# marcemq/crowdmod-ddpm-4D

Hardware: AMD Instinct MI355X
Metric: denoise-steps/sec (UNet fwd + sampler update) at ATC [B,4,T,H,W] (higher is better)
Workload: dtype f32; 1 GPU; config/ATC.yml sampling on the 12x36 grid, fp32 arithmetic (fp32 matrix instructions; fp32 products built from f16 two-way splits -- three v_mfma_f32_32x32x16_f16 cross terms, fp32 accumulate, same error against the reference as round 3's six-term bf16 form -- in the Winograd / quarter-resolution / last-conv layers, whose input is GroupNorm + SiLU output, and in the upsample layers, whose raw inpu; channels=4, past_len=5, future_len=3, global_batch=64, parallelism=batch-shard x1 (2 stream lanes of 32 chains per rank)

## Files before the change

### crowdmod-ddpm-4d_amd/csrc/cm_attn_block.hip

```cpp
#include "cm_kernels.h"

#include <algorithm>

namespace cm {

typedef float f32x4 __attribute__((ext_vector_type(4)));

constexpr int ATT_NT = 768;
constexpr int ATT_KS = 3;

template <int D>
__global__ __launch_bounds__(ATT_NT) void attn_head_kernel(const AttnBlockArgs a) {
  constexpr int NT = ATT_NT, NW = NT / 64;
  constexpr int KD = D < 16 ? 16 : D;
  constexpr int DS = KD + 4;
  constexpr int NBQ = (D + 15) / 16;
  constexpr int NBT = 3 * NBQ;
  constexpr int PARTS = D / 8;
  constexpr int E = 4 * D;
  constexpr int XS = E + 8;
  constexpr int Q4 = E >> 2;
  constexpr int RL = NT / Q4;
  extern __shared__ __attribute__((aligned(16))) float sm[];
  const int S = a.S;
  float *Xs = sm;
  float *Wi = Xs + (size_t)S * XS;
  float *Wo = Wi + (size_t)NBT * 16 * XS;
  float *Qs = Wo + (size_t)E * DS;
  float *Ks = Qs + (size_t)S * DS;
  float *Vs = Ks + (size_t)S * DS;
  float *bi = Vs + (size_t)S * DS;
  float *red = bi + NBT * 16;
  const int h = blockIdx.x, b = blockIdx.y, tid = threadIdx.x;
  const int lane = tid & 63, wave = __builtin_amdgcn_readfirstlane(tid >> 6);
  const int r16 = lane & 15, kq = lane >> 4;

  const int q4 = tid % Q4, rl = tid / Q4;
  const float *xb = a.x + (size_t)b * S * E;
  constexpr int UX = 3;
  constexpr int NWI = (NBT * 16 + RL - 1) / RL;
  constexpr int NWO = (E * (KD / 4) + NT - 1) / NT;
  f32x4 vx[UX], vwi[NWI], vwo[NWO];
#pragma unroll
  for (int u = 0; u < UX; ++u) vx[u] = *reinterpret_cast<const f32x4 *>(xb + (size_t)min(rl + u * RL, S - 1) * E + 4 * q4);
#pragma unroll
  for (int u = 0; u < NWI; ++u) {
    const int wr = min(rl + u * RL, NBT * 16 - 1);
    const int which = wr / (NBQ * 16), c = min(wr % (NBQ * 16), D - 1);
    vwi[u] = *reinterpret_cast<const f32x4 *>(a.w_in + (size_t)(which * E + h * D + c) * E + 4 * q4);
  }
#pragma unroll
  for (int u = 0; u < NWO; ++u) {
    const int i = min(tid + u * NT, E * (KD / 4) - 1);
    const int n = i / (KD / 4), c4 = min(i % (KD / 4), D / 4 - 1);
    vwo[u] = *reinterpret_cast<const f32x4 *>(a.w_out + (size_t)n * E + h * D + 4 * c4);
  }
  const f32x4 ga = *reinterpret_cast<const f32x4 *>(a.gamma + 4 * q4);
  const f32x4 be = *reinterpret_cast<const f32x4 *>(a.beta + 4 * q4);
  float bval = 0.f;
  {
    const int tb = min(tid, NBT * 16 - 1);
    const int which = tb / (NBQ * 16), c = min(tb % (NBQ * 16), D - 1);
    bval = a.b_in[which * E + h * D + c];
  }
  float s1 = 0.f;
#pragma unroll
  for (int u = 0; u < UX; ++u) {
    const int row = rl + u * RL;
    if (row < S) {
      *reinterpret_cast<f32x4 *>(Xs + row * XS + 4 * q4) = vx[u];
      s1 += (vx[u][0] + vx[u][1]) + (vx[u][2] + vx[u][3]);
    }
  }
#pragma unroll
  for (int u = 0; u < NWI; ++u) {
    const int wr = rl + u * RL;
    if (wr < NBT * 16) *reinterpret_cast<f32x4 *>(Wi + wr * XS + 4 * q4) = vwi[u];
  }
#pragma unroll
  for (int u = 0; u < NWO; ++u) {
    const int i = tid + u * NT;
    if (i < E * (KD / 4)) {
      const int n = i / (KD / 4), c4 = i % (KD / 4);
      *reinterpret_cast<f32x4 *>(Wo + n * DS + 4 * c4) = (4 * c4 < D) ? vwo[u] : f32x4{0.f, 0.f, 0.f, 0.f};
    }
// ... 133 lines not shown
        float L = 0.f;
        f32x4 O0 = {0.f, 0.f, 0.f, 0.f}, O1 = {0.f, 0.f, 0.f, 0.f};
#pragma unroll
        for (int s2i = 0; s2i < ATT_KS; ++s2i) {
          const float *mp = mrg + ((prow * ATT_KS + s2i) * PARTS + part) * 12;
          const float w = (mp[1] > 0.f) ? __expf(mp[0] - M) : 0.f;
          L += mp[1] * w;
          O0 += *reinterpret_cast<const f32x4 *>(mp + 4) * w;
          O1 += *reinterpret_cast<const f32x4 *>(mp + 8) * w;
        }
        const float inv = 1.0f / L;
        *reinterpret_cast<f32x4 *>(Qs + row * DS + 8 * part) = O0 * inv;
        *reinterpret_cast<f32x4 *>(Qs + row * DS + 8 * part + 4) = O1 * inv;
      }
      __syncthreads();
    }
  }

  {
    constexpr int NJ = KD / 16;
    constexpr int nbe = E >> 4;
    float *pout = a.part + ((size_t)h * a.B + b) * (size_t)S * E;
    for (int item = wave; item < nmb * nbe; item += NW) {
      const int mb = item / nbe, nb = item - mb * nbe;
      const int arow = min(mb * 16 + r16, S - 1);
      f32x4 af[NJ], bf[NJ];
#pragma unroll
      for (int j = 0; j < NJ; ++j) {
        af[j] = *reinterpret_cast<const f32x4 *>(Qs + arow * DS + 16 * j + 4 * kq);
        bf[j] = *reinterpret_cast<const f32x4 *>(Wo + (nb * 16 + r16) * DS + 16 * j + 4 * kq);
      }
      f32x4 acc = {0.f, 0.f, 0.f, 0.f};
#pragma unroll
      for (int j = 0; j < NJ; ++j)
#pragma unroll
        for (int jj = 0; jj < 4; ++jj) acc = __builtin_amdgcn_mfma_f32_16x16x4f32(af[j][jj], bf[j][jj], acc, 0, 0, 0);
      const int n = nb * 16 + r16;
#pragma unroll
      for (int reg = 0; reg < 4; ++reg) {
        const int row = mb * 16 + 4 * kq + reg;
        if (row < S) pout[(size_t)row * E + n] = acc[reg];
      }
    }
  }
}

size_t attn_block_lds_bytes(int S, int E, int heads) {
  const int D = E / heads, KD = D < 16 ? 16 : D, NBT = 3 * ((D + 15) / 16);
  return ((size_t)S * (E + 8) + (size_t)NBT * 16 * (E + 8) + (size_t)E * (KD + 4) + (size_t)3 * S * (KD + 4) + (size_t)NBT * 16 +
          (size_t)(ATT_NT / (E / 4)) * 8 + 8) * sizeof(float);
}

bool attn_block_ok(int S, int E, int heads, int groups) {
  if (heads != 4 || E % heads) return false;
  const int D = E / heads;
  if (D != 8 && D != 16 && D != 32) return false;
  if (groups != 8 || E % (4 * groups)) return false;
  return S >= 1 && attn_block_lds_bytes(S, E, heads) <= 160 * 1024;
}

hipError_t launch_attn_block(const AttnBlockArgs &a, hipStream_t st) {
  if (!attn_block_ok(a.S, a.E, a.heads, a.groups)) return hipErrorInvalidValue;
  const int D = a.E / a.heads;
  const size_t smem = attn_block_lds_bytes(a.S, a.E, a.heads);
#define CM_ATTNB(DD)                                                                                        \
  if (D == DD) {                                                                                            \
    static bool attr_set[64] = {false};                                                                     \
    int dev = 0;                                                                                            \
    (void)hipGetDevice(&dev);                                                                               \
    if (!attr_set[dev & 63]) {                                                                              \
      hipError_t e = hipFuncSetAttribute(reinterpret_cast<const void *>(attn_head_kernel<DD>),              \
                                         hipFuncAttributeMaxDynamicSharedMemorySize, 160 * 1024);           \
      if (e != hipSuccess) return e;                                                                        \
      attr_set[dev & 63] = true;                                                                            \
    }                                                                                                       \
    hipLaunchKernelGGL((attn_head_kernel<DD>), dim3(a.heads, a.B), dim3(ATT_NT), smem, st, a);                 \
    return hipGetLastError();                                                                               \
  }
  CM_ATTNB(8) CM_ATTNB(16) CM_ATTNB(32)
#undef CM_ATTNB
  return hipErrorInvalidValue;
}

}
```

### crowdmod-ddpm-4d_amd/csrc/cm_kernels.h

```cpp
#pragma once
#include <hip/hip_runtime.h>
#include <stdint.h>
#include <stdlib.h>
#include <vector>

namespace cm {

inline const char *diag_env(const char *name) {
  static const bool on = [] { const char *d = getenv("CM_DIAG"); return d && d[0] == '1' && d[1] == 0; }();
  return on ? getenv(name) : nullptr;
}

#ifdef __HIPCC__
typedef float cm_f32x2_t __attribute__((ext_vector_type(2)));
typedef float cm_f32x4_t __attribute__((ext_vector_type(4)));
typedef __bf16 cm_bf16x2_t __attribute__((ext_vector_type(2)));
typedef unsigned cm_u32x2_t __attribute__((ext_vector_type(2)));
typedef _Float16 cm_f16x4_t __attribute__((ext_vector_type(4)));
__device__ __forceinline__ unsigned cm_cvt_pk_bf16(float a, float b) {
  const cm_f32x2_t v = {a, b};
  return __builtin_bit_cast(unsigned, __builtin_convertvector(v, cm_bf16x2_t));
}
template <int NT = 3>
__device__ __forceinline__ void cm_split3_bf16(cm_f32x4_t x, cm_u32x2_t (&t)[3]) {
// ... 213 lines not shown
  float h2_oscale;
  const float *wq;
  const float *bias;
  const float *temb;
  int temb_stride;
  const long long *tidx;
  const float *resid;
  int res_cs;
  float *out;
  int out_cs, Co, B, Y, X;
  float *stat_part, *stat_cnt;
  int stat_C;
  const float *s2src0, *s2src1;
  int s2C0, s2C1;
  const float *s2w;
  int qshift;
  const float *pm;
  int pm_stride;
  int raw;
};
bool conv_qr_ok(const QrArgs &a);
bool conv_qr2_b6_ok(const QrArgs &a);
hipError_t launch_qr_b6_repack(const float *wq, float *wq6, long long n_floats, int Ci, hipStream_t st);
hipError_t launch_conv_qr(const QrArgs &a, hipStream_t st);

bool conv_f16d_pick(int Z, int Y, int X, int *bz, int *by, int *bx, int *mbw);
bool conv_f16d_ok(const ConvArgs &a, int mbw);
int conv_f16d_slots(const ConvArgs &a, int mbw);
hipError_t launch_conv_f16d(const ConvArgs &a, int mbw, hipStream_t st);

bool conv_fin_pick(int Y, int X, int *by, int *bx);
bool conv_fin_ok(const ConvArgs &a);
struct StepArgs;
bool conv_fin_fuse_ok(const ConvArgs &a, const StepArgs &s);
hipError_t launch_conv_fin(const ConvArgs &a, const float *wfin, int mode , hipStream_t st,
                           const StepArgs *step = nullptr, int variant = 1);
inline int conv_first_const_ztiles(int bz, int ntz, int P) {
  if (bz < 1 || P < 2 || (P - 1) % bz) return 0;
  const int n = (P - 1) / bz;
  return n < ntz ? n : 0;
}
hipError_t launch_fin_pack(const float *w_ref , float *wfin, int Co, int mode , hipStream_t st, float wscale = 1.f);
constexpr size_t CM_FIN_W_FLOATS = 4 * 2 * 3 * 64 * 4;

hipError_t launch_chan_stats(const float *x, int B, int V, int C, int nslice, float *part, float *cnt, hipStream_t st);
hipError_t launch_gn_finalize(const float *part0, const float *cnt0, int ns0, int C0, const float *part1,
                              const float *cnt1, int ns1, int C1, int V, const float *gamma, const float *beta,
                              int groups, float eps, float *gn, float *mr, int B, hipStream_t st);
struct CombineArgs {
  const float *part; int S; long long stride;
  const float *bias; const float *temb; int temb_stride; const long long *tidx;
  const float *resid; int res_cs;
  float *out; int C, V, B;
  float *stat_part; float *stat_cnt; int nslots;
  const float *fin_gamma, *fin_beta; float *fin_gn, *fin_mr;
  const float *fin_p1, *fin_n1; int fin_ns1, fin_C1, fin_groups; float fin_eps;
};
hipError_t launch_ksplit_combine(const CombineArgs &a, hipStream_t st);
bool combine_gn_ok(const CombineArgs &a);
hipError_t launch_combine_gn(const CombineArgs &a, hipStream_t st);
hipError_t launch_assemble_input(const float *past, const float *future, float *x8, int B, int C, int H, int W,
                                 int P, int F, int which , hipStream_t st);
hipError_t launch_extract_output(const float *eps_cl, int cs, float *out, int B, int C, int H, int W, int P, int F,
                                 hipStream_t st);
hipError_t launch_time_mlp(const float *table, const float *W1, const float *b1, const float *W2, const float *b2,
                           const float *Wd, const float *bd, int te, int tx, int nproj, int nrows, float *temb_raw,
                           float *out, const long long *rowidx, hipStream_t st);
hipError_t launch_attn_core(const float *qkv, float *out, int B, int S, int E, int heads, hipStream_t st);
hipError_t launch_attn_core_f16(const float *qkv, float *out, int B, int S, int E, int heads, hipStream_t st);

struct AttnBlockArgs {
  const float *x;
  const float *gamma, *beta;
  const float *w_in, *b_in;
  const float *w_out;
  float *part;
  int B, S, E, heads, groups;
  float eps;
};
bool attn_block_ok(int S, int E, int heads, int groups);
size_t attn_block_lds_bytes(int S, int E, int heads);
hipError_t launch_attn_block(const AttnBlockArgs &a, hipStream_t st);

enum { DIT_PRO_NONE = 0, DIT_PRO_LN = 1, DIT_PRO_PATCH = 2 };
enum { DIT_EPI_BIAS = 0, DIT_EPI_SILU = 1, DIT_EPI_SILU2 = 2, DIT_EPI_GELU = 3, DIT_EPI_GATE = 4, DIT_EPI_PATCH = 5,
       DIT_EPI_UNPATCH = 6 };
struct DitGemmArgs {
  int pro, epi;
  const float *A; int lda;
  const float *W, *bias;
  float *Y; int ldy;
  long long M; int N, K;
  int grp, grp_stride, grp_off;
  int a_compact;
  int tok;
  const long long *tbuf;
  const float *mod; int ldmod;
  int off_shift, off_scale, off_gate;
  const float *x8;
  const float *spos, *tpos;
  int L, Hh, Ww, p, pt, Ns, wpn, Cout;
};
struct DitAttnArgs {
  const float *qkv;
  float *out;
  int B, Tp, Ns, qs, E, heads;
};
hipError_t launch_dit_gemm(const DitGemmArgs &a, hipStream_t st);
hipError_t launch_dit_attn_spatial(const DitAttnArgs &a, hipStream_t st);
hipError_t launch_dit_attn_temporal(const DitAttnArgs &a, hipStream_t st);
hipError_t launch_dit_attn_full(const DitAttnArgs &a, hipStream_t st);

struct StepRow { int t; float c_x, c_eps, c_noise, guid; int draw; int step; float mass; };
struct StepArgs {
  float *x;
  const float *eps_cl;
  int cs;
  float *x8;
  const float *noise;
  float *hist;
  int B, C, H, W, P, F;
  float c_x, c_eps, c_noise;
  float guid;
  unsigned long long seed;
  long long sample_id_base;
  int step;
  int draw;
  const StepRow *tab; const int *kctr;
  long long row_stride;
  long long boff;
  long long *t_next; long long t_next_v;
};
hipError_t launch_sampler_step(const StepArgs &a, hipStream_t st);
#ifdef __HIPCC__
__device__ __forceinline__ void philox4x32_10(unsigned c0, unsigned c1, unsigned c2, unsigned c3, unsigned k0,
                                              unsigned k1, unsigned out[4]) {
#pragma unroll
  for (int i = 0; i < 10; ++i) {
    const unsigned long long p0 = 0xD2511F53ull * c0;
    const unsigned long long p1 = 0xCD9E8D57ull * c2;
    const unsigned n0 = (unsigned)(p1 >> 32) ^ c1 ^ k0;
    const unsigned n1 = (unsigned)p1;
    const unsigned n2 = (unsigned)(p0 >> 32) ^ c3 ^ k1;
    const unsigned n3 = (unsigned)p0;
    c0 = n0; c1 = n1; c2 = n2; c3 = n3;
    k0 += 0x9E3779B9u;
    k1 += 0xBB67AE85u;
  }
  out[0] = c0; out[1] = c1; out[2] = c2; out[3] = c3;
}

__device__ __forceinline__ float philox_normal(unsigned long long seed, long long sample, int step, long long elem) {
  unsigned r[4];
  philox4x32_10((unsigned)(elem >> 1), (unsigned)sample, (unsigned)step, (unsigned)((sample >> 32) ^ 0x5eed),
                (unsigned)seed, (unsigned)(seed >> 32), r);
  const float u1 = ((float)(r[0] >> 8) + 0.5f) * (1.0f / 16777216.0f);
  const float u2 = ((float)(r[1] >> 8) + 0.5f) * (1.0f / 16777216.0f);
  const float rad = sqrtf(-2.0f * __logf(u1));
  const float ang = 6.283185307179586f * u2;
  return (elem & 1) ? rad * __sinf(ang) : rad * __cosf(ang);
}

__device__ __forceinline__ void cm_step_resolve(StepArgs &a) {
  if (a.tab) {
    const int k = *a.kctr;
    const StepRow r = a.tab[k];
// ... 132 lines not shown
```

### crowdmod-ddpm-4d_amd/csrc/cm_model.cpp

```cpp
#include <hip/hip_runtime.h>

#include <algorithm>
#include <cmath>
#include <cstdarg>
#include <cstdio>
#include <cstring>
#include <map>
#include <memory>
#include <set>
#include <string>
#include <thread>
#include <vector>

#include "../../include/crowdmod_hip.h"
#include "cm_kernels.h"

namespace {

thread_local std::string g_err;

int fail(const char *fmt, ...) {
  char buf[1024];
  va_list ap;
  va_start(ap, fmt);
// ... 47 lines not shown
  std::string prefix;
  int cin, cout, attention, skip, level;
};

enum OpKind { OP_CONV, OP_STATS, OP_GNFIN, OP_ATTN, OP_ATTNBLK };

struct Op {
  OpKind kind;
  int cls;
  cm::ConvArgs ca{};
  int MB = 1, NB = 1;
  int *d_hvtab = nullptr, *d_mtab = nullptr;
  Act *stat_act = nullptr;
  int pm_off = -1;
  const Act *in0 = nullptr, *in1 = nullptr;
  std::string wname, bname;
  int temb_off = -1;
  int gn_op = -1;
  int ref_taps = 1;
  int ks = 1;
  const Act *skip0 = nullptr, *skip1 = nullptr;
  std::string skip_w, skip_b;
  float *d_s2w = nullptr, *d_bias_fused = nullptr;
  bool skip_if_fused = false;
  bool wino = false;
  float *d_wwino = nullptr;
  float *d_wwino16 = nullptr;
  float *d_wwino_b6 = nullptr;
  long long wwino_floats = 0;
  float *d_wfrag16 = nullptr;
  float *d_w1x1_16 = nullptr;
  long long wpar_stride16 = 0;
  bool f16d = false;
  int f16d_bz = 0, f16d_by = 0, f16d_bx = 0, f16d_mbw = 0;
  bool ups = false;
  int ups_tz = 0, ups_ty = 0, ups_tx = 0, ups_mbw = 0, ups_planes = 0;
  float *d_wups16 = nullptr;
  long long wups16_stride = 0;
  float *d_wups_b6 = nullptr;
  long long wups_b6_stride = 0;
  float *d_w16d = nullptr, *d_w16d_skip = nullptr;
  bool h2_off = false;
  bool dbg_h2 = false;
  bool dbg_raw = false;
  float *d_wfin_h2 = nullptr, *d_wwino_h2 = nullptr, *d_wqr_h2 = nullptr;
  float *d_wups_h2 = nullptr;
  float h2_oscale = 1.f;
  bool qr = false;
  float *d_wqr = nullptr, *d_wqr_skip = nullptr;
  float *d_wqr_b6 = nullptr;
  bool train_qr = false;
  long long wqr_floats = 0;
  bool qr_consumer = false;
  bool first_k = false;
  int first_cin = 4;
  float *d_wfirst = nullptr;
  bool small_n = false;
  float *d_wsmall = nullptr;
  int small_nco = 4;
  bool fin = false;
  int fin_by = 0, fin_bx = 0;
  float *d_wfin = nullptr, *d_wfin16 = nullptr, *d_wfin_src = nullptr;
  float *d_zero_bias = nullptr;
  const Act *out_act = nullptr, *resid_act = nullptr;
  double flops_per_sample = 0;
  std::string label;
  double prof_ms = 0;
  int64_t prof_n = 0;
  const Act *act = nullptr;
  const Act *g0 = nullptr, *g1 = nullptr;
  const float *gamma = nullptr, *beta = nullptr;
  float *gn_out = nullptr;
  float *gn_mr = nullptr;
  std::string gname, bename;
  const float *qkv = nullptr;
  float *aout = nullptr;
  int S = 0, E = 0;
  bool in_attn_block = false;
  const Act *ab_x = nullptr;
  Act *ab_out = nullptr;
  int ab_gn = -1, ab_qkv = -1, ab_outc = -1;
  float *d_win = nullptr, *d_wout = nullptr;
  std::string win_name, wout_name;
};

enum ConvKernel { CONV_NONE, CONV_QR, CONV_KSPLIT, CONV_UPS, CONV_F16D, CONV_WINO, CONV_FIRST, CONV_FIN, CONV_SMALLN, CONV_1X1_F16, CONV_GENERIC };
const char *const kConvKernelName[] = {"none", "qr", "ksplit", "ups", "f16d", "wino", "first", "fin", "smalln", "1x1_f16", "generic"};
enum ConvForm { FORM_FP32 = 0, FORM_F16 = 1, FORM_B6 = 2, FORM_B3 = 3, FORM_H2 = 4 };
struct ConvRoute { ConvKernel kernel; ConvForm form; };

struct FwdCtx { int precision = CM_PRECISION_F32; bool train_fwd = false, h2_stale = false; int B = 1; };
enum FinBy { FIN_NONE, FIN_QR, FIN_COMBINE, FIN_WINO, FIN_ALONE };
struct OpPlan {
  bool launch = false;
  ConvRoute route{CONV_NONE, FORM_FP32};
  int ns_out = 0;
  int ns0 = 0, ns1 = 0;
  FinBy fin = FIN_NONE;
  int carries = -1;
};
struct FwdPlan { FwdCtx ctx; std::vector<OpPlan> ops; std::string err; };

}

struct cm_schedule {
  int T = 0;
  int device = 0;
  std::vector<float> tab[6];
  float *d_sab = nullptr, *d_s1m = nullptr;
};

struct cm_train_state;
struct cm_dit_plan;
void cm_free_train_state(cm_train_state *t);
struct cm_model {
  cm_unet_config cfg{};
  cm_dit_plan *dit = nullptr;
  int device = 0;
  hipStream_t stream = nullptr;
  hipStream_t lane_stream[4] = {nullptr, nullptr, nullptr, nullptr};
  hipEvent_t ev_join[4] = {nullptr, nullptr, nullptr, nullptr}, ev_fork = nullptr;
  std::vector<Param> params;
  std::map<std::string, int> pindex;
  std::vector<BlockDesc> enc, bott, dec;
  int final_ch = 0;
  bool finalized = false;
  int precision = CM_PRECISION_F32;

  std::vector<void *> allocs;
  std::vector<std::unique_ptr<Act>> acts;
  std::map<std::string, Act *> act_by_name;
  std::vector<Op> ops;
  FwdPlan plan;
  std::map<std::string, float *> dparam;

  float *x8 = nullptr;
  Act *x8_act = nullptr;
  float *eps_cl = nullptr;
  long long *tbuf = nullptr;
  float *temb_table = nullptr;
  int nproj = 0;
  float *d_time[7] = {nullptr};
  struct cm_train_state *train = nullptr;
  float *dropmask = nullptr;
  bool h2_stale = false;
  float *train_temb = nullptr;
  long long *train_iota = nullptr;
  bool use_train_temb = false;
  float *mse_partial = nullptr, *mse_loss = nullptr;
  float *ks_scratch = nullptr;
  size_t ks_scratch_floats = 0;
  float *xstate = nullptr;
  cm::StepRow *d_steptab = nullptr;
  size_t steptab_cap = 0;
  int *d_kctr = nullptr;
  int *d_nonfinite = nullptr;
  int loop_ends = cm::diag_env("CM_LOOP_ENDS") ? (atoi(cm::diag_env("CM_LOOP_ENDS")) & 15) : 7;
  float *mass_q = nullptr;
  float *stage_past = nullptr, *stage_fut = nullptr, *stage_out = nullptr;
  float *stage_noise = nullptr;
  size_t stage_noise_cap = 0;
  float *stage_hist = nullptr;
  size_t stage_hist_cap = 0;

  bool profile = false;
  float prof_ms[K_NCLASS] = {0};
  int64_t prof_n[K_NCLASS] = {0};
  std::vector<std::pair<int, std::pair<hipEvent_t, hipEvent_t>>> prof_events[4];
  hipEvent_t prof_base = nullptr;
  int prof_B = 0;
  float prof_union_ms[8] = {0, 0, 0, 0, 0, 0, 0, 0};

  int L() const { return cfg.past_len + cfg.future_len; }
  int64_t per_sample() const { return (int64_t)cfg.in_channels * cfg.rows * cfg.cols * cfg.future_len; }
};

namespace {
int refresh_h2(cm_model *m);

void add_param(cm_model *m, const std::string &name, std::vector<int64_t> shape) {
  Param p;
  p.name = name;
// ... 150 lines not shown
  const uint32_t sign = (uint32_t)(h & 0x8000u) << 16;
  uint32_t exp = (h >> 10) & 0x1fu, man = h & 0x3ffu, x;
  if (exp == 0) {
    if (man == 0) { x = sign; }
    else {
      int e = -1;
      do { ++e; man <<= 1; } while (!(man & 0x400u));
      x = sign | ((uint32_t)(127 - 15 - e) << 23) | ((man & 0x3ffu) << 13);
    }
  } else if (exp == 31) {
    x = sign | 0x7f800000u | (man << 13);
  } else {
    x = sign | ((exp + 127 - 15) << 23) | (man << 13);
  }
  float f;
  std::memcpy(&f, &x, 4);
  return f;
}

std::vector<float> pack_conv_weights_f16(const float *W, int Co, int Ci, int ntaps, int Ci_pad, int CK, int NB) {
  const int TN = 32 * NB, ntn = (Co + TN - 1) / TN, nch = Ci_pad / CK, K8 = CK / 8, nsteps = ntaps * K8;
  std::vector<uint16_t> out((size_t)ntn * nch * nsteps * NB * 64 * 4, 0);
  size_t o = 0;
  for (int nt = 0; nt < ntn; ++nt)
    for (int ch = 0; ch < nch; ++ch)
      for (int s = 0; s < nsteps; ++s) {
        const int t = s / K8, j = s % K8;
        for (int nb = 0; nb < NB; ++nb)
          for (int lane = 0; lane < 64; ++lane)
            for (int jj = 0; jj < 4; ++jj, ++o) {
              const int co = nt * TN + nb * 32 + (lane & 31);
              const int ci = ch * CK + 8 * j + 4 * (lane >> 5) + jj;
              if (co < Co && ci < Ci) out[o] = f32_to_f16_bits(W[((size_t)co * Ci + ci) * ntaps + t]);
            }
      }
  std::vector<float> packed(out.size() / 2);
  std::memcpy(packed.data(), out.data(), out.size() * 2);
  return packed;
}

std::vector<float> pack_ups_f16(const float *W, int Co, int Ci) {
  const int ncb = Co / 32, nch = Ci / 32;
  std::vector<uint16_t> out((size_t)ncb * nch * 8 * 2 * 64 * 8, 0);
  size_t o = 0;
  for (int cb = 0; cb < ncb; ++cb)
    for (int ch = 0; ch < nch; ++ch)
      for (int t = 0; t < 8; ++t)
        for (int mg = 0; mg < 2; ++mg)
          for (int lane = 0; lane < 64; ++lane)
            for (int i = 0; i < 8; ++i, ++o) {
              const int co = cb * 32 + (lane & 31), ci = ch * 32 + 16 * mg + 8 * (lane >> 5) + i;
              out[o] = f32_to_f16_bits(W[((size_t)co * Ci + ci) * 8 + t]);
            }
  std::vector<float> packed(out.size() / 2);
  std::memcpy(packed.data(), out.data(), out.size() * 2);
  return packed;
}

static inline uint16_t f32_to_bf16_bits(float f) {
  uint32_t u;
  std::memcpy(&u, &f, 4);
  if ((u & 0x7fffffffu) > 0x7f800000u) return (uint16_t)((u >> 16) | 0x40);
  u += 0x7fffu + ((u >> 16) & 1u);
  return (uint16_t)(u >> 16);
}
static inline float bf16_bits_to_f32(uint16_t h) {
  const uint32_t u = (uint32_t)h << 16;
  float f;
  std::memcpy(&f, &u, 4);
  return f;
}
static inline void f16_split2(float w, float scale, uint16_t out[3]) {
  const float v = w * scale;
  out[0] = f32_to_f16_bits(v);
  out[1] = f32_to_f16_bits(v - f16_bits_to_f32(out[0]));
  out[2] = 0;
}
static inline void bf16_split3(float w, uint16_t out[3]) {
  float rem = w;
  for (int t = 0; t < 3; ++t) {
    out[t] = f32_to_bf16_bits(rem);
    rem -= bf16_bits_to_f32(out[t]);
  }
}

std::vector<float> pack_ups_b6(const float *W, int Co, int Ci, float h2_scale = 0.f) {
  const int ncb = Co / 32, nch = Ci / 32;
  std::vector<uint16_t> out((size_t)ncb * nch * 8 * 2 * 3 * 64 * 8, 0);
  for (int cb = 0; cb < ncb; ++cb)
    for (int ch = 0; ch < nch; ++ch)
      for (int t = 0; t < 8; ++t)
        for (int mg = 0; mg < 2; ++mg)
          for (int lane = 0; lane < 64; ++lane)
            for (int i = 0; i < 8; ++i) {
              const int co = cb * 32 + (lane & 31), ci = ch * 32 + 16 * mg + 8 * (lane >> 5) + i;
              uint16_t t3[3];
              if (h2_scale > 0.f) f16_split2(W[((size_t)co * Ci + ci) * 8 + t], h2_scale, t3);
              else bf16_split3(W[((size_t)co * Ci + ci) * 8 + t], t3);
              for (int tm = 0; tm < 3; ++tm)
                out[(((((((size_t)cb * nch + ch) * 8 + t) * 2 + mg) * 3 + tm) * 64) + lane) * 8 + i] = t3[tm];
            }
  std::vector<float> packed(out.size() / 2);
  std::memcpy(packed.data(), out.data(), out.size() * 2);
  return packed;
}

std::vector<float> pack_conv_weights(const float *W, int Co, int Ci, int ntaps, int Ci_pad, int CK, int NB) {
  const int TN = 32 * NB, ntn = (Co + TN - 1) / TN, nch = Ci_pad / CK, K8 = CK / 8, nsteps = ntaps * K8;
  std::vector<float> out((size_t)ntn * nch * nsteps * NB * 64 * 4, 0.f);
  size_t o = 0;
  for (int nt = 0; nt < ntn; ++nt)
    for (int ch = 0; ch < nch; ++ch)
      for (int s = 0; s < nsteps; ++s) {
        const int t = s / K8, j = s % K8;
        for (int nb = 0; nb < NB; ++nb)
          for (int lane = 0; lane < 64; ++lane)
            for (int jj = 0; jj < 4; ++jj, ++o) {
              const int co = nt * TN + nb * 32 + (lane & 31);
              const int ci = ch * CK + 8 * j + 4 * (lane >> 5) + jj;
              if (co < Co && ci < Ci) out[o] = W[((size_t)co * Ci + ci) * ntaps + t];
            }
      }
  return out;
}

void pack_wino(const std::vector<float> *wi, const std::vector<int> *ii, int Co, int Ci, int Ci_pad, std::vector<float> *out,
               std::vector<int> *oidx, std::vector<float> *ocoef) {
  static const double G[4][3] = {{1, 0, 0}, {0.5, 0.5, 0.5}, {0.5, -0.5, 0.5}, {0, 0, 1}};
  const int ntn = (Co + 31) / 32, nch = Ci_pad / 16;
  const size_t total = (size_t)ntn * nch * 4 * 24 * 64 * 4;
  if (out) out->assign(total, 0.f);
  if (oidx) { oidx->assign(total * 9, -1); ocoef->assign(total * 9, 0.f); }
  for (int co = 0; co < Co; ++co)
    for (int ci = 0; ci < Ci; ++ci)
      for (int dz = 0; dz < 3; ++dz)
        for (int xy = 0; xy < 4; ++xy)
          for (int xx = 0; xx < 4; ++xx) {
            const int nt = co / 32, r = co % 32, chunk = ci / 16, k8 = (ci % 16) / 8, hh = (ci % 8) / 4, jj = ci % 4;
            const size_t o = ((((((size_t)nt * nch + chunk) * 4 + xy) * 24 + (dz * 2 + k8) * 4 + xx) * 64) + hh * 32 + r) * 4 + jj;
            double acc = 0;
            for (int dy = 0; dy < 3; ++dy)
              for (int dx = 0; dx < 3; ++dx) {
                const size_t t = ((size_t)co * Ci + ci) * 27 + (dz * 3 + dy) * 3 + dx;
                const double c = G[xy][dy] * G[xx][dx];
                if (wi) acc += c * (double)(*wi)[t];
                if (oidx && c != 0.0) { (*oidx)[o * 9 + dy * 3 + dx] = (*ii)[t]; (*ocoef)[o * 9 + dy * 3 + dx] = (float)c; }
              }
            if (out) (*out)[o] = (float)acc;
          }
}

uint16_t f32_to_f16_bits(float f) {
  uint32_t x;
  std::memcpy(&x, &f, 4);
  const uint32_t sign = (x >> 16) & 0x8000u;
  const int32_t exp = (int32_t)((x >> 23) & 0xff) - 127 + 15;
  uint32_t man = x & 0x7fffffu;
  if (((x >> 23) & 0xff) == 0xff) return (uint16_t)(sign | 0x7c00u | (man ? 0x200u : 0));
  if (exp >= 31) return (uint16_t)(sign | 0x7c00u);
  if (exp <= 0) {
    if (exp < -10) return (uint16_t)sign;
    man |= 0x800000u;
    const int shift = 14 - exp;
    uint32_t h = man >> shift;
    const uint32_t rem = man & ((1u << shift) - 1), half = 1u << (shift - 1);
    if (rem > half || (rem == half && (h & 1))) ++h;
// ... 216 lines not shown
  return out;
}
std::vector<float> pack_qr_b6(const std::vector<float> &wq, int Co, int Ci, float h2_scale = 0.f) {
  const int ntn = Co / 32, K8 = Ci / 8, ng = 9 * K8, cw = Ci / 8, nsw = (cw + 15) / 16;
  std::vector<uint16_t> out((size_t)ntn * 8 * nsw * 9 * 3 * 3 * 64 * 8, 0);
  for (size_t i = 0; i < wq.size(); ++i) {
    const int jj = (int)(i & 3), lane = (int)((i >> 2) & 63);
    size_t q = i >> 8;
    const int dz = (int)(q % 3); q /= 3;
    const int g = (int)(q % ng);
    const int nt = (int)(q / ng);
    const int k8 = g / 9, t9 = g % 9, ci = 8 * k8 + 4 * (lane >> 5) + jj, r = lane & 31;
    const int wv = ci / cw, cl = ci % cw, st = cl / 16, hd = (cl % 16) / 8, j = cl % 8;
    uint16_t t3[3];
    if (h2_scale > 0.f) f16_split2(wq[i], h2_scale, t3);
    else bf16_split3(wq[i], t3);
    for (int tm = 0; tm < 3; ++tm)
      out[(((((((size_t)(nt * 8 + wv) * nsw + st) * 9 + t9) * 3 + dz) * 3 + tm) * 64) + 32 * hd + r) * 8 + j] = t3[tm];
  }
  std::vector<float> packed(out.size() / 2);
  std::memcpy(packed.data(), out.data(), out.size() * 2);
  return packed;
}
std::vector<float> pack_qr_skip(const float *w2, int Co, int Cs) {
  const int ntn = Co / 32, ngs = Cs / 8;
  std::vector<float> out((size_t)ntn * ngs * 64 * 4, 0.f);
  size_t o = 0;
  for (int nt = 0; nt < ntn; ++nt)
    for (int gs = 0; gs < ngs; ++gs)
      for (int lane = 0; lane < 64; ++lane)
        for (int jj = 0; jj < 4; ++jj, ++o)
          out[o] = w2[(size_t)(nt * 32 + (lane & 31)) * Cs + 8 * gs + 4 * (lane >> 5) + jj];
  return out;
}

static float h2_wscale(const float *w, size_t n) {
  float mx = 0.f;
  for (size_t i = 0; i < n; ++i) mx = std::max(mx, std::fabs(w[i]));
  if (!(mx > 0.f) || !std::isfinite(mx)) return 0.f;
  int e = 0;
  (void)std::frexp(mx, &e);
  return std::ldexp(1.0f, 13 - e);
}
static bool h2_bound_ok(const std::vector<float> &g, const std::vector<float> &b, const Op &gop, double gain);
static bool h2_act_bounded(const cm_model *m, const Op &gop, double gain) {
  return h2_bound_ok(P(m, gop.gname).host, P(m, gop.bename).host, gop, gain);
}
static bool h2_bound_ok(const std::vector<float> &g, const std::vector<float> &b, const Op &gop, double gain) {
  double gm = 0, bm = 0;
  for (float v : g) gm = std::max(gm, (double)std::fabs(v));
  for (float v : b) bm = std::max(bm, (double)std::fabs(v));
  const int Ct = gop.g0->C + (gop.g1 ? gop.g1->C : 0);
  const double n = (double)(Ct / GN_GROUPS) * gop.g0->V();
  const double bound = (std::sqrt(n) * gm + bm) * gain;
  return std::isfinite(bound) && bound <= 32000.0;
}

static float h2_pack_wino(const float *w_ref, int Co, int Ci_ref, int Ci_pad, std::vector<float> *out) {
  const std::vector<float> wi = to_internal_taps(w_ref, Co, Ci_ref, 27);
  std::vector<float> ww;
  pack_wino(&wi, nullptr, Co, Ci_ref, Ci_pad, &ww, nullptr, nullptr);
  const float ws = h2_wscale(ww.data(), ww.size());
  if (ws > 0.f) *out = pack_wino_b6(ww, ws);
  return ws;
}
static float h2_pack_qr(const float *w_ref, int Co, int Ci_ref, std::vector<float> *out) {
  const std::vector<float> wq = pack_qr(to_internal_taps(w_ref, Co, Ci_ref, 27), Co, Ci_ref);
  const float ws = h2_wscale(wq.data(), wq.size());
  if (ws > 0.f) *out = pack_qr_b6(wq, Co, Ci_ref, ws);
  return ws;
}
static float h2_pack_ups(const float *w_ref, int Co, int Ci_ref, std::vector<float> *out) {
  const std::vector<float> wp = parity_weights(to_internal_taps(w_ref, Co, Ci_ref, 27), Co, Ci_ref);
  const size_t per = (size_t)Co * Ci_ref * 8;
  const float ws = h2_wscale(wp.data(), wp.size());
  if (ws > 0.f) {
    out->clear();
    for (int p8 = 0; p8 < 8; ++p8) {
      const std::vector<float> one = pack_ups_b6(wp.data() + p8 * per, Co, Ci_ref, ws);
      out->insert(out->end(), one.begin(), one.end());
    }
  }
  return ws;
}

int add_conv(cm_model *m, const ConvSpec &s) {
  Op op;
  op.kind = OP_CONV;
  op.cls = s.ntaps == 27 ? K_CONV3 : K_CONV1;
  cm::ConvArgs &a = op.ca;
  a.src0 = s.s0->d; a.C0 = s.s0->C;
  a.src1 = s.s1 ? s.s1->d : nullptr; a.C1 = s.s1 ? s.s1->C : 0;
  a.gn = s.gn; a.silu = s.silu;
  a.Zs = s.s0->Z; a.Ys = s.s0->Y; a.Xs = s.s0->X;
  a.Zo = s.out->Z; a.Yo = s.out->Y; a.Xo = s.out->X;
  a.ntaps = s.ntaps; a.stride = s.stride; a.ups = s.ups;
  a.td = s.ntaps == 27 ? 3 : 1; a.par = 0; a.wpar_stride = 0;
  const bool parity = s.ups && s.ntaps == 27 && !cm::diag_env("CM_NO_PARITY_UPCONV");
  if (parity) { a.ups = 0; a.par = 1; a.td = 2; a.ntaps = 8; }
  a.out = s.out->d; a.out_cs = s.out->C; a.Co = s.Co;
  a.temb = s.temb; a.temb_stride = m->nproj; a.tidx = m->tbuf;
  a.resid = s.resid ? s.resid->d : nullptr; a.res_cs = s.resid ? s.resid->C : 0;
  a.CK = pick_ck(a.C0, a.C1);
  if (s.ntaps == 1) {
    for (int ck : {256, 128, 64})
      if (a.C0 % ck == 0 && a.C1 % ck == 0) { a.CK = ck; break; }
  }
  if (!a.CK) return fail("conv %s: channel counts %d/%d not multiples of 8", s.wname.c_str(), a.C0, a.C1);
  a.nch0 = a.C0 / a.CK; a.nch1 = a.C1 / a.CK;
  op.NB = s.Co > 32 ? 2 : 1;
  {
    int wz = 0, wy = 0, wx = 0;
    op.wino = s.ntaps == 27 && s.stride == 1 && !s.ups && a.C0 % 16 == 0 && a.C1 % 16 == 0 && s.Co % 32 == 0 && s.Co == s.out->C &&
              s.ci_valid < 0 && s.out->V() > 64 && cm::conv_wino_pick(s.out->Z, s.out->Y, s.out->X, &wz, &wy, &wx) && !cm::diag_env("CM_NO_WINO");
  }
  if (s.ntaps == 27 && s.out->V() <= 64 && cm::diag_env("CM_QR_NB")) op.NB = atoi(cm::diag_env("CM_QR_NB"));
  if (op.wino) op.NB = 1;
  if (s.ntaps == 27 && s.out->V() > 64 && !op.wino) {
    if (const TunedTile *t = find_tuned(a, 0)) op.NB = t->NB;
    if (s.Co == 64 && cm::diag_env("CM_NB64")) op.NB = atoi(cm::diag_env("CM_NB64"));
    if (s.Co == 128 && cm::diag_env("CM_NB128")) op.NB = atoi(cm::diag_env("CM_NB128"));
  }
  const Param &w = P(m, s.wname);
  const Param &b = P(m, s.bname);
  const int Ci_ref = (int)w.shape[1];
  const int Ci_pad = a.C0 + a.C1;
  if (Ci_ref > Ci_pad || (s.ci_valid < 0 && Ci_ref != Ci_pad))
    return fail("conv %s: weight has %d input channels, sources provide %d", s.wname.c_str(), Ci_ref, Ci_pad);
  const std::vector<float> wi = to_internal_taps(w.host.data(), (int)w.shape[0], Ci_ref, s.ntaps);
  std::vector<float> wf;
  if (parity) {
    const std::vector<float> wp = parity_weights(wi, (int)w.shape[0], Ci_ref);
    const size_t per = (size_t)w.shape[0] * Ci_ref * 8;
    for (int p8 = 0; p8 < 8; ++p8) {
      std::vector<float> one = pack_conv_weights(wp.data() + p8 * per, (int)w.shape[0], Ci_ref, 8, Ci_pad, a.CK, op.NB);
      a.wpar_stride = (long long)one.size();
      wf.insert(wf.end(), one.begin(), one.end());
    }
    if (m->precision == CM_PRECISION_F16 && a.CK == 32) {
      std::vector<float> wf16;
      for (int p8 = 0; p8 < 8; ++p8) {
        std::vector<float> one = pack_conv_weights_f16(wp.data() + p8 * per, (int)w.shape[0], Ci_ref, 8, Ci_pad, a.CK, op.NB);
        op.wpar_stride16 = (long long)one.size();
        wf16.insert(wf16.end(), one.begin(), one.end());
      }
      if (upload(m, wf16, &op.d_wfrag16)) return 1;
    }
  } else {
    wf = pack_conv_weights(wi.data(), (int)w.shape[0], Ci_ref, s.ntaps, Ci_pad, a.CK, op.NB);
    if (m->precision == CM_PRECISION_F16 && s.ntaps == 1 && s.stride == 1 && !s.ups && !s.stats && !s.temb && Ci_ref == Ci_pad &&
        a.C0 % 16 == 0 && a.C1 % 16 == 0 && !cm::diag_env("CM_NO_1X1_F16") &&
        upload(m, pack_1x1_f16(wi.data(), (int)w.shape[0], Ci_ref, op.NB), &op.d_w1x1_16))
      return 1;
  }
  if (parity && a.CK == 32 && !s.s1 && !s.gn && !s.temb && !s.resid && s.Co % 32 == 0 && s.Co == s.out->C && !cm::diag_env("CM_NO_UPS") &&
      cm::conv_ups_pick(a.Zs, a.Ys, a.Xs, &op.ups_tz, &op.ups_ty, &op.ups_tx, &op.ups_mbw, &op.ups_planes) &&
      (a.Zs / op.ups_tz) * (a.Ys / op.ups_ty) * (a.Xs / op.ups_tx) * 8 * op.ups_mbw <= MAX_SLOTS)
    op.ups = true;
  if (op.ups && m->precision != CM_PRECISION_F16 && Ci_ref == Ci_pad && Ci_ref % 32 == 0 && !cm::diag_env("CM_NO_UPS_B6")) {
    const std::vector<float> wp = parity_weights(wi, (int)w.shape[0], Ci_ref);
    const size_t per = (size_t)w.shape[0] * Ci_ref * 8;
    std::vector<float> wb6;
    for (int p8 = 0; p8 < 8; ++p8) {
      const std::vector<float> one = pack_ups_b6(wp.data() + p8 * per, (int)w.shape[0], Ci_ref);
      op.wups_b6_stride = (long long)one.size();
      wb6.insert(wb6.end(), one.begin(), one.end());
// ... 227 lines not shown
    auto visit = [&](const BlockDesc &b) { if (b.kind == 0) { temb_off[b.prefix] = off; off += b.cout; } };
    for (auto &b : m->enc) visit(b);
    for (auto &b : m->bott) visit(b);
    for (auto &b : m->dec) visit(b);
    m->nproj = off;
  }
  if (dev_alloc(m, (void **)&m->temb_table, (size_t)TIME_ROWS * m->nproj * sizeof(float))) return 1;

  auto xin = std::make_unique<Act>();
  xin->name = "input"; xin->C = 8; xin->Z = L; xin->Y = c.rows; xin->X = c.cols;
  if (dev_alloc(m, (void **)&xin->d, (size_t)c.max_batch * xin->V() * 8 * sizeof(float))) return 1;
  CM_HIP(hipMemset(xin->d, 0, (size_t)c.max_batch * xin->V() * 8 * sizeof(float)));
  m->x8 = xin->d; m->x8_act = xin.get();
  m->acts.push_back(std::move(xin));

  auto res_block = [&](const BlockDesc &b, const Act *x0, const Act *x1, Act **result) -> int {
    const int l = b.level;
    const std::string &p = b.prefix;
    float *gn1 = nullptr, *gn2 = nullptr;
    if (add_gnfin(m, x0, x1, p + ".normalize_1.weight", p + ".normalize_1.bias", &gn1)) return 1;
    Act *h1 = new_act(m, p + ".conv_1", b.cout, Zl[l], Yl[l], Xl[l], true, &rc);
    if (rc) return 1;
    ConvSpec c1; c1.s0 = x0; c1.s1 = x1; c1.gn = gn1; c1.silu = 1; c1.wname = p + ".conv_1.weight"; c1.bname = p + ".conv_1.bias";
    c1.temb = m->temb_table + temb_off[p]; c1.out = h1; c1.Co = b.cout; c1.stats = true;
    if (add_conv(m, c1)) return 1;
    add_stats(m, h1);
    if (add_gnfin(m, h1, nullptr, p + ".normalize_2.weight", p + ".normalize_2.bias", &gn2)) return 1;
    const Act *resid = x0;
    int mi_index = -1;
    if (b.cin != b.cout) {
      Act *r = new_act(m, p + ".match_input", b.cout, Zl[l], Yl[l], Xl[l], false, &rc);
      if (rc) return 1;
      ConvSpec cs; cs.s0 = x0; cs.s1 = x1; cs.ntaps = 1; cs.wname = p + ".match_input.weight"; cs.bname = p + ".match_input.bias";
      cs.out = r; cs.Co = b.cout;
      if (add_conv(m, cs)) return 1;
      mi_index = (int)m->ops.size() - 1;
      resid = r;
    } else if (x1) {
      return fail("identity skip with concatenated input is not expressible (block %s)", p.c_str());
    }
    Act *h2 = new_act(m, b.attention ? p + ".conv_2+skip" : p, b.cout, Zl[l], Yl[l], Xl[l], true, &rc);
    if (rc) return 1;
    ConvSpec c2; c2.s0 = h1; c2.gn = gn2; c2.silu = 1; c2.wname = p + ".conv_2.weight"; c2.bname = p + ".conv_2.bias";
    c2.resid = resid; c2.out = h2; c2.Co = b.cout; c2.stats = true; c2.pm_off = temb_off[p];
    if (mi_index >= 0) { c2.skip0 = x0; c2.skip1 = x1; c2.skip_w = p + ".match_input.weight"; c2.skip_b = p + ".match_input.bias"; }
    if (add_conv(m, c2)) return 1;
    if (mi_index >= 0 && m->ops.back().d_s2w) m->ops[mi_index].skip_if_fused = true;
    add_stats(m, h2);
    *result = h2;
    if (b.attention) {
      const std::string ap = p + ".attention";
      float *gna = nullptr;
      if (add_gnfin(m, h2, nullptr, ap + ".group_norm.weight", ap + ".group_norm.bias", &gna)) return 1;
      Act *qkv = new_act(m, ap + ".qkv", 3 * b.cout, Zl[l], Yl[l], Xl[l], false, &rc);
      if (rc) return 1;
      ConvSpec cq; cq.s0 = h2; cq.gn = gna; cq.silu = 0; cq.ntaps = 1; cq.wname = ap + ".mhsa.in_proj_weight"; cq.bname = ap + ".mhsa.in_proj_bias";
      cq.out = qkv; cq.Co = 3 * b.cout;
      if (add_conv(m, cq)) return 1;
      Act *ao = new_act(m, ap + ".core", b.cout, Zl[l], Yl[l], Xl[l], false, &rc);
      if (rc) return 1;
      Op at; at.kind = OP_ATTN; at.cls = K_ATTN; at.label = ap + ".core"; at.qkv = qkv->d; at.aout = ao->d; at.S = qkv->V(); at.E = b.cout;
      if ((size_t)2 * at.S * (at.E / ATTN_HEADS) * 4 > 160 * 1024)
        return fail("attention with %d tokens exceeds the LDS-resident K/V design", at.S);
      m->ops.push_back(at);
      Act *h3 = new_act(m, p, b.cout, Zl[l], Yl[l], Xl[l], true, &rc);
      if (rc) return 1;
      ConvSpec co; co.s0 = ao; co.ntaps = 1; co.wname = ap + ".mhsa.out_proj.weight"; co.bname = ap + ".mhsa.out_proj.bias";
      co.resid = h2; co.out = h3; co.Co = b.cout; co.stats = true;
      if (add_conv(m, co)) return 1;
      add_stats(m, h3);
      *result = h3;
      const int nops = (int)m->ops.size();
      if (cm::attn_block_ok(qkv->V(), b.cout, ATTN_HEADS, GN_GROUPS) && !cm::diag_env("CM_NO_FUSED_ATTN") && !cm::diag_env("CM_NO_FUSED_STATS")) {
        Op fb;
        fb.kind = OP_ATTNBLK; fb.cls = K_ATTN; fb.label = ap + " (fused block)";
        fb.ab_x = h2; fb.ab_out = h3; fb.S = qkv->V(); fb.E = b.cout;
        fb.ab_gn = nops - 4; fb.ab_qkv = nops - 3; fb.ab_outc = nops - 1;
        if (m->ops[fb.ab_gn].kind != OP_GNFIN || m->ops[fb.ab_qkv].kind != OP_CONV || m->ops[nops - 2].kind != OP_ATTN ||
            m->ops[fb.ab_outc].kind != OP_CONV)
          return fail("attention block plan out of order");
        fb.win_name = ap + ".mhsa.in_proj_weight"; fb.wout_name = ap + ".mhsa.out_proj.weight";
        if (upload(m, P(m, fb.win_name).host, &fb.d_win)) return 1;
        if (upload(m, P(m, fb.wout_name).host, &fb.d_wout)) return 1;
        for (int i = nops - 4; i < nops; ++i) m->ops[i].in_attn_block = true;
        const size_t need = (size_t)ATTN_HEADS * m->cfg.max_batch * fb.S * fb.E;
        m->ks_scratch_floats = std::max(m->ks_scratch_floats, need);
        m->ops.push_back(fb);
      }
    }
    return 0;
  };

  Act *h = new_act(m, "first", c.base_channels, Zl[0], Yl[0], Xl[0], true, &rc);
  if (rc) return 1;
  {
    ConvSpec cf; cf.s0 = m->x8_act; cf.wname = "first.weight"; cf.bname = "first.bias"; cf.out = h; cf.Co = c.base_channels; cf.ci_valid = c.in_channels; cf.stats = true;
    if (add_conv(m, cf)) return 1;
    add_stats(m, h);
  }
  std::vector<Act *> outs{h};
  for (auto &b : m->enc) {
    if (b.kind == 0) {
      Act *r = nullptr;
      if (res_block(b, h, nullptr, &r)) return 1;
      h = r;
    } else {
      Act *d = new_act(m, b.prefix, b.cout, Zl[b.level + 1], Yl[b.level + 1], Xl[b.level + 1], true, &rc);
      if (rc) return 1;
      ConvSpec cd; cd.s0 = h; cd.stride = 2; cd.wname = b.prefix + ".downsample.weight"; cd.bname = b.prefix + ".downsample.bias"; cd.out = d; cd.Co = b.cout; cd.stats = true;
      if (add_conv(m, cd)) return 1;
      add_stats(m, d);
      h = d;
    }
    outs.push_back(h);
  }
  for (auto &b : m->bott) {
    Act *r = nullptr;
    if (res_block(b, h, nullptr, &r)) return 1;
    h = r;
  }
  for (auto &b : m->dec) {
    if (b.kind == 0) {
      Act *skip = outs.back();
      outs.pop_back();
      Act *r = nullptr;
      if (res_block(b, h, skip, &r)) return 1;
      h = r;
    } else {
      const int l = b.level - 1;
      Act *u = new_act(m, b.prefix, b.cout, Zl[l], Yl[l], Xl[l], true, &rc);
      if (rc) return 1;
      ConvSpec cu; cu.s0 = h; cu.ups = 1; cu.wname = b.prefix + ".upsample.1.weight"; cu.bname = b.prefix + ".upsample.1.bias"; cu.out = u; cu.Co = b.cout; cu.stats = true;
      if (add_conv(m, cu)) return 1;
      add_stats(m, u);
      h = u;
    }
  }
  {
    float *gnf = nullptr;
    if (add_gnfin(m, h, nullptr, "final.0.weight", "final.0.bias", &gnf)) return 1;
    auto eo = std::make_unique<Act>();
    eo->name = "final"; eo->C = 8; eo->Z = L; eo->Y = c.rows; eo->X = c.cols;
    if (dev_alloc(m, (void **)&eo->d, (size_t)c.max_batch * eo->V() * 8 * sizeof(float))) return 1;
    CM_HIP(hipMemset(eo->d, 0, (size_t)c.max_batch * eo->V() * 8 * sizeof(float)));
    m->eps_cl = eo->d;
    Act *eop = eo.get();
    m->act_by_name["final"] = eop;
    m->acts.push_back(std::move(eo));
    ConvSpec cf; cf.s0 = h; cf.gn = gnf; cf.silu = 1; cf.wname = "final.2.weight"; cf.bname = "final.2.bias"; cf.out = eop; cf.Co = c.out_channels;
    if (add_conv(m, cf)) return 1;
  }
  if (m->ks_scratch_floats && dev_alloc(m, (void **)&m->ks_scratch, 4 * m->ks_scratch_floats * sizeof(float))) return 1;
  return 0;
}

int resolve_conv(cm_model *m, Op &op) {
  if (op.wino) {
    cm::ConvArgs a = op.ca;
    a.bs = 1;
    op.wino = cm::conv_wino_pick(a.Zo, a.Yo, a.Xo, &a.bz, &a.by, &a.bx);
    if (op.wino) {
      a.ntz = a.Zo / a.bz; a.nty = (a.Yo + a.by - 1) / a.by; a.ntx = (a.Xo + a.bx - 1) / a.bx;
      op.wino = cm::conv_wino_ok(a);
    }
    if (op.wino) {
      op.ca = a;
// ... 66 lines not shown
  }
  if (op.d_w1x1_16 && infer && cm::conv1x1_f16_ok(a, op.NB)) return {CONV_1X1_F16, FORM_F16};
  return {CONV_GENERIC, form(cm::conv_par_f16_variant(op.MB, op.NB, g.bz, g.by, g.bx) ? op.d_wfrag16 : nullptr, nullptr, nullptr)};
}

bool route_takes_h16(ConvRoute r, int mask) {
  switch (r.kernel) {
    case CONV_F16D: return true;
    case CONV_UPS: return r.form == FORM_F16 && !(mask & ~5);
    case CONV_FIRST: return !(mask & ~4);
    case CONV_FIN: case CONV_SMALLN: return !(mask & ~3);
    default: return false;
  }
}

struct LoopEnds {
  int tz_first = 0;
  int zo_first = 0, zo_end = 0;
  int fuse = 0;
  const cm::StepArgs *step = nullptr;
};
LoopEnds loop_ends_plan(const std::vector<Op> &ops, const float *x8, const float *eps_cl, int mask, int precision, bool h2_stale, int P, int F,
                        int Cin, int Cout) {
  LoopEnds le;
  for (const Op &op : ops) {
    if (op.kind != OP_CONV) continue;
    const ConvRoute r = conv_route(op, precision, false, h2_stale);
    if (r.kernel == CONV_FIRST && op.ca.src0 == x8 && (mask & 4)) le.tz_first = cm::conv_first_const_ztiles(op.ca.bz, op.ca.ntz, P);
    if (r.kernel == CONV_FIN && op.ca.out == eps_cl && op.ca.Zo == P + F && (mask & 3)) {
      le.zo_first = P; le.zo_end = P + F;
      if ((mask & 2) && Cin == Cout && op.ca.Co == Cout && op.ca.out_cs == 8 && F <= 8) le.fuse = (mask & 8) ? 2 : 1;
    }
  }
  return le;
}

int plan_h16(cm_model *m) {
  if (m->precision != CM_PRECISION_F16 || cm::diag_env("CM_NO_H16")) return 0;
  auto takes = [&](const Op &o, int role) { return route_takes_h16(conv_route(o, m->precision, false, false), role); };
  for (auto &ap : m->acts) {
    Act *a = ap.get();
    bool ok = false;
    for (const Op &o : m->ops)
      if (o.kind == OP_CONV && o.out_act == a && !o.skip_if_fused) ok = takes(o, 4);
    for (const Op &o : m->ops) {
      if (!ok) break;
      if (o.kind == OP_ATTNBLK && o.ab_x == a) ok = false;
      if (o.kind == OP_ATTN && (o.qkv == a->d || o.aout == a->d)) ok = false;
      if (o.kind != OP_CONV || o.skip_if_fused) continue;
      const int role = (o.in0 == a ? 1 : 0) | (o.in1 == a ? 2 : 0) | (o.resid_act == a ? 8 : 0) | (o.skip0 == a ? 16 : 0) | (o.skip1 == a ? 32 : 0);
      if (role) ok = takes(o, role);
    }
    a->h16 = ok;
  }
  return 0;
}

std::string plan_conv(const Op &op, const FwdCtx &ctx, int src_slots, OpPlan *p) {
  ConvRoute r = conv_route(op, ctx.precision, ctx.train_fwd, ctx.h2_stale);
  if (r.kernel == CONV_UPS && r.form == FORM_H2 && src_slots <= 0) {
    Op plain = op; plain.d_wups_h2 = nullptr;
    r = conv_route(plain, ctx.precision, ctx.train_fwd, ctx.h2_stale);
  }
  p->route = r; p->launch = r.kernel != CONV_NONE; p->ns_out = 0; p->ns0 = src_slots;
  const int h16 = h16_mask(op, ctx.train_fwd);
  if (p->launch && h16 && r.kernel != CONV_QR && !route_takes_h16(r, h16))
    return "conv " + op.label + ": f16 tensors (mask " + std::to_string(h16) + ") reach a kernel without f16 tensor support";
  if (!p->launch || !op.stat_act) return "";
  cm::ConvArgs a = op.ca;
  int ns = a.ntz * a.nty * a.ntx * op.MB * (a.par ? 8 : 1);
  if (r.kernel == CONV_QR) ns = a.Yo * a.Xo > 32 ? 4 : 2;
  if (r.kernel == CONV_KSPLIT) ns = (a.Zo * a.Yo * a.Xo + 31) / 32;
  if (r.kernel == CONV_UPS) { a.bz = op.ups_tz; a.by = op.ups_ty; a.bx = op.ups_tx; ns = cm::conv_ups_slots(a, op.ups_mbw); }
  if (r.kernel == CONV_F16D) { a.bz = op.f16d_bz; a.by = op.f16d_by; a.bx = op.f16d_bx; ns = cm::conv_f16d_slots(a, op.f16d_mbw); }
  if (ns < 1 || ns > MAX_SLOTS) return "conv " + op.label + ": " + std::to_string(ns) + " statistics slots, outside [1, " + std::to_string(MAX_SLOTS) + "]";
  p->ns_out = ns;
  return "";
}

bool wino_merges(const Op &c, ConvRoute r, int B) {
  cm::ConvArgs a = c.ca;
  a.B = B; a.f16 = r.form == FORM_F16 ? a.f16 : (int)r.form;
  return r.kernel == CONV_WINO && r.form != FORM_FP32 && a.gn && cm::conv_wino_p_taken(a, r.form == FORM_F16, true);
}

FwdPlan plan_forward(const std::vector<Op> &ops, const FwdCtx &ctx) {
  static const bool no_fuse = cm::diag_env("CM_NO_FUSE_GNFIN") != nullptr, no_slot_gn = cm::diag_env("CM_NO_SLOT_GN") != nullptr;
  FwdPlan P{ctx, std::vector<OpPlan>(ops.size()), ""};
  const bool infer = !ctx.train_fwd; const int n = (int)ops.size();
  std::map<const Act *, int> slots;
  auto slots_of = [&](const Act *t) { return slots.count(t) ? slots[t] : 0; };
  auto in_ctx = [&](const Op &o) { return o.kind == OP_ATTNBLK ? infer : !(o.in_attn_block && infer); };
  for (int i = 0; i < n && P.err.empty(); ++i) {
    const Op &op = ops[i];
    OpPlan &p = P.ops[i];
    if (!in_ctx(op)) continue;
    p.launch = op.kind != OP_GNFIN;
    const Act *two_pass = nullptr; int pc = 0, pv = 0;
    if (op.kind == OP_CONV) {
      P.err = plan_conv(op, ctx, (op.in0 && op.in0->part) ? slots_of(op.in0) : 0, &p);
      if (p.ns_out) slots[op.stat_act] = p.ns_out;
      if (p.route.kernel == CONV_KSPLIT) { two_pass = op.stat_act; pc = op.ca.Co; pv = op.ca.Zo * op.ca.Yo * op.ca.Xo; }
    } else if (op.kind == OP_STATS) {
      slots[op.act] = p.ns_out = op.act->nslice;
    } else if (op.kind == OP_ATTNBLK) {
      slots[op.ab_out] = p.ns_out = (op.S + 31) / 32; two_pass = op.ab_out; pc = op.E; pv = op.S;
    } else if (op.kind == OP_GNFIN && p.fin != FIN_COMBINE) {
      p.ns0 = slots_of(op.g0); p.ns1 = op.g1 ? slots_of(op.g1) : 0;
      if (p.ns0 < 1 || (op.g1 && p.ns1 < 1)) P.err = op.label + ": no earlier op of the forward writes its statistics";
      int cons = -1, ncons = 0;
      for (int j = i + 1; j < n; ++j) if (ops[j].kind == OP_CONV && ops[j].gn_op == i) { cons = j; ++ncons; }
      const bool merge = ncons == 1 && infer && !no_slot_gn && p.ns0 <= 16 && (!op.g1 || (p.ns1 <= 16 && op.g1->V() == op.g0->V())) &&
                         wino_merges(ops[cons], conv_route(ops[cons], ctx.precision, false, ctx.h2_stale), ctx.B);
      p.fin = (op.qr_consumer && infer) ? FIN_QR : merge ? FIN_WINO : FIN_ALONE; p.launch = p.fin == FIN_ALONE;
    }
    int j = i + 1;
    while (j < n && !in_ctx(ops[j])) ++j;
    if (!two_pass || no_fuse || j == n || ops[j].kind != OP_GNFIN || ops[j].g0 != two_pass || (ops[j].qr_consumer && infer)) continue;
    const Act *g1 = ops[j].g1;
    cm::CombineArgs cb{};
    cb.C = pc; cb.V = pv; cb.B = ctx.B; cb.nslots = p.ns_out; cb.stat_part = two_pass->part; cb.fin_C1 = g1 ? g1->C : 0; cb.fin_groups = GN_GROUPS;
    if ((g1 && (g1->V() != pv || slots_of(g1) < 1)) || !cm::combine_gn_ok(cb)) continue;
    p.carries = j; P.ops[j].fin = FIN_COMBINE; P.ops[j].ns0 = p.ns_out; P.ops[j].ns1 = g1 ? slots_of(g1) : 0;
  }
  return P;
}

int build_time_table(cm_model *m) {
  const cm_unet_config &c = m->cfg;
  const int te = c.base_channels, tx = c.base_channels * c.time_multiple;
  std::vector<float> Wd((size_t)m->nproj * tx), bd((size_t)m->nproj);
  int off = 0;
  auto visit = [&](const BlockDesc &b) {
    if (b.kind != 0) return;
    const Param &w = P(m, b.prefix + ".dense_1.weight");
    const Param &bb = P(m, b.prefix + ".dense_1.bias");
    std::copy(w.host.begin(), w.host.end(), Wd.begin() + (size_t)off * tx);
    std::copy(bb.host.begin(), bb.host.end(), bd.begin() + off);
    off += b.cout;
  };
  for (auto &b : m->enc) visit(b);
  for (auto &b : m->bott) visit(b);
  for (auto &b : m->dec) visit(b);
  float *dT, *dW1, *db1, *dW2, *db2, *dWd, *dbd;
  if (upload(m, P(m, "time_embeddings.time_blocks.0.weight").host, &dT)) return 1;
  if (upload(m, P(m, "time_embeddings.time_blocks.1.weight").host, &dW1)) return 1;
  if (upload(m, P(m, "time_embeddings.time_blocks.1.bias").host, &db1)) return 1;
  if (upload(m, P(m, "time_embeddings.time_blocks.3.weight").host, &dW2)) return 1;
  if (upload(m, P(m, "time_embeddings.time_blocks.3.bias").host, &db2)) return 1;
  if (upload(m, Wd, &dWd)) return 1;
  if (upload(m, bd, &dbd)) return 1;
  m->d_time[0] = dT; m->d_time[1] = dW1; m->d_time[2] = db1; m->d_time[3] = dW2; m->d_time[4] = db2;
  m->d_time[5] = dWd; m->d_time[6] = dbd;
  CM_HIP(cm::launch_time_mlp(dT, dW1, db1, dW2, db2, dWd, dbd, te, tx, m->nproj, TIME_ROWS, nullptr, m->temb_table, nullptr, m->stream));
  CM_HIP(hipStreamSynchronize(m->stream));
  return 0;
}

float *slot_part(const Act *t, int ns, int b0) { return t->part + (size_t)b0 * ns * t->C * 2; }
float *slot_cnt(const Act *t, int ns, int b0) { return t->cnt + (size_t)b0 * ns; }

int run_gnfin(const Op &g, const OpPlan &gp, int B, hipStream_t st, int b0) {
  const Act *g0 = g.g0, *g1 = g.g1; const int Ct = g0->C + (g1 ? g1->C : 0);
  if (g1 && g1->V() != g0->V()) return fail("concat sources disagree on voxel count");
  CM_HIP(cm::launch_gn_finalize(slot_part(g0, gp.ns0, b0), slot_cnt(g0, gp.ns0, b0), gp.ns0, g0->C,
                                g1 ? slot_part(g1, gp.ns1, b0) : nullptr, g1 ? slot_cnt(g1, gp.ns1, b0) : nullptr,
                                g1 ? gp.ns1 : 0, g1 ? g1->C : 0, g0->V(), g.gamma, g.beta, GN_GROUPS, GN_EPS,
                                g.gn_out + (size_t)b0 * 2 * Ct, g.gn_mr ? g.gn_mr + (size_t)b0 * 2 * Ct : nullptr, B, st));
  return 0;
}

int run_combine(cm::CombineArgs &cb, const std::vector<Op> &ops, const FwdPlan &plan, int fin, int b0, hipStream_t st) {
  if (fin >= 0) {
    const Op &f = ops[fin];
    const Act *g1 = f.g1;
    const int Ct = cb.C + (g1 ? g1->C : 0), ns1 = plan.ops[fin].ns1;
    cb.fin_gamma = f.gamma; cb.fin_beta = f.beta;
    cb.fin_gn = f.gn_out + (size_t)b0 * 2 * Ct; cb.fin_mr = f.gn_mr ? f.gn_mr + (size_t)b0 * 2 * Ct : nullptr;
    if (g1) { cb.fin_p1 = slot_part(g1, ns1, b0); cb.fin_n1 = slot_cnt(g1, ns1, b0); cb.fin_ns1 = ns1; cb.fin_C1 = g1->C; }
    cb.fin_groups = GN_GROUPS; cb.fin_eps = GN_EPS;
  }
  CM_HIP(fin >= 0 ? cm::launch_combine_gn(cb, st) : cm::launch_ksplit_combine(cb, st));
  return 0;
}

int run_conv_qr(const cm_model *m, const Op &op, const FwdPlan &plan, const OpPlan &p, hipStream_t st, int b0) {
  const Op &gop = m->ops[op.gn_op]; const OpPlan &gp = plan.ops[op.gn_op];
  const Act *g0 = gop.g0, *g1 = gop.g1;
  const cm::ConvArgs &ca = op.ca;
  const bool train = plan.ctx.train_fwd; const size_t V = (size_t)ca.Zo * ca.Yo * ca.Xo;
  cm::QrArgs q{};
  q.src0 = ca.src0 + (size_t)b0 * V * ca.C0; q.C0 = ca.C0;
  q.src1 = ca.src1 ? ca.src1 + (size_t)b0 * V * ca.C1 : nullptr; q.C1 = ca.C1;
  q.part0 = slot_part(g0, gp.ns0, b0); q.cnt0 = slot_cnt(g0, gp.ns0, b0); q.ns0 = gp.ns0;
  if (g1) { q.part1 = slot_part(g1, gp.ns1, b0); q.cnt1 = slot_cnt(g1, gp.ns1, b0); q.ns1 = gp.ns1; }
  if (g0->C != ca.C0 || (g1 ? g1->C : 0) != ca.C1) return fail("quarter-resolution conv %s: statistics and sources disagree", op.label.c_str());
  q.gamma = gop.gamma; q.beta = gop.beta; q.groups = GN_GROUPS; q.eps = GN_EPS; q.silu = ca.silu;
  if (op.dbg_raw) { q.gamma = q.beta = nullptr; q.raw = 1; q.silu = 0; }
  q.wq = op.d_wqr; q.bias = ca.bias;
  q.wq6 = op.d_wqr_b6;
  q.three = p.route.form == FORM_B3 ? 1 : 0;
  if (p.route.form == FORM_H2) { q.wq6 = op.d_wqr_h2; q.three = 2; q.h2_oscale = op.h2_oscale; }
  q.temb = ca.temb; q.temb_stride = ca.temb_stride; q.tidx = ca.tidx + b0;
  q.resid = ca.resid ? ca.resid + (size_t)b0 * V * ca.res_cs : nullptr; q.res_cs = ca.res_cs;
  if (train) {
    if (op.pm_off >= 0) { q.pm = m->dropmask + (size_t)b0 * m->nproj + op.pm_off; q.pm_stride = m->nproj; }
// ... 42 lines not shown
  if (op.stat_act) {
    ca.stat_C = op.stat_act->C; ca.stat_ns = p.ns_out;
    ca.stat_part = slot_part(op.stat_act, p.ns_out, b0); ca.stat_cnt = slot_cnt(op.stat_act, p.ns_out, b0);
  }
  switch (route.kernel) {
    case CONV_NONE: case CONV_QR: break;
    case CONV_KSPLIT: {
      cm::ConvArgs ka = ca;
      const int V = op.out_act->V();
      float *scratch = m->ks_scratch + (size_t)slab * m->ks_scratch_floats;
      ka.temb = nullptr; ka.resid = nullptr; ka.stat_part = nullptr; ka.bias = op.d_zero_bias;
      ka.out = scratch; ka.out_cs = ka.Co;
      ka.ks = op.ks; ka.kpart = (long long)B * V * ka.Co;
      CM_HIP(cm::launch_conv(ka, op.MB, op.NB, st));
      cm::CombineArgs cb{};
      cb.part = scratch; cb.S = op.ks; cb.stride = ka.kpart;
      cb.bias = ca.bias; cb.temb = ca.temb; cb.temb_stride = ca.temb_stride; cb.tidx = ca.tidx;
      cb.resid = ca.resid; cb.res_cs = ca.res_cs;
      cb.out = ca.out; cb.C = ka.Co; cb.V = V; cb.B = B;
      cb.nslots = p.ns_out; cb.stat_part = ca.stat_part; cb.stat_cnt = ca.stat_cnt;
      return run_combine(cb, m->ops, plan, p.carries, b0, st);
    }
    case CONV_UPS:
      if (route.form == FORM_F16) { ca.wfrag = op.d_wups16; ca.wpar_stride = op.wups16_stride; }
      else if (route.form != FORM_FP32) { ca.wfrag = op.d_wups_b6; ca.wpar_stride = op.wups_b6_stride; }
      ca.f16 = route.form;
      if (route.form == FORM_H2) {
        ca.wfrag = op.d_wups_h2; ca.h2_oscale = op.h2_oscale;
        ca.gp0 = slot_part(op.in0, p.ns0, b0); ca.gc0 = slot_cnt(op.in0, p.ns0, b0); ca.gns0 = p.ns0;
      }
      ca.bz = op.ups_tz; ca.by = op.ups_ty; ca.bx = op.ups_tx;
      ca.ntz = ca.Zs / ca.bz; ca.nty = ca.Ys / ca.by; ca.ntx = ca.Xs / ca.bx;
      CM_HIP(cm::launch_conv_ups(ca, op.ups_mbw, op.ups_planes, op.NB, st));
      break;
    case CONV_F16D:
      ca.bz = op.f16d_bz; ca.by = op.f16d_by; ca.bx = op.f16d_bx;
      ca.wfrag = op.d_w16d;
      if (ca.s2w) ca.s2w = op.d_w16d_skip;
      CM_HIP(cm::launch_conv_f16d(ca, op.f16d_mbw, st));
      break;
    case CONV_WINO: {
      const bool f16 = route.form == FORM_F16;
      ca.wfrag = f16 ? op.d_wwino16 : route.form == FORM_H2 ? op.d_wwino_h2 : route.form == FORM_FP32 ? op.d_wwino : op.d_wwino_b6;
      if (!f16) ca.f16 = route.form;
      if (route.form == FORM_H2) ca.h2_oscale = op.h2_oscale;
      if (ca.gn && op.gn_op >= 0 && plan.ops[op.gn_op].fin == FIN_WINO) {
        const Op &g = m->ops[op.gn_op]; const OpPlan &gp = plan.ops[op.gn_op];
        ca.gp0 = slot_part(g.g0, gp.ns0, b0); ca.gc0 = slot_cnt(g.g0, gp.ns0, b0); ca.gns0 = gp.ns0;
        if (g.g1) { ca.gp1 = slot_part(g.g1, gp.ns1, b0); ca.gc1 = slot_cnt(g.g1, gp.ns1, b0); ca.gns1 = gp.ns1; }
        ca.gs_gamma = g.gamma; ca.gs_beta = g.beta; ca.gs_groups = GN_GROUPS; ca.gs_eps = GN_EPS; ca.gn = nullptr;
      }
      CM_HIP(cm::launch_conv_wino(ca, f16, st));
      break;
    }
    case CONV_FIRST:
      if (le && op.ca.src0 == m->x8) ca.tz_first = le->tz_first;
      CM_HIP(cm::launch_conv_first(ca, op.first_cin, op.d_wfirst, st));
      break;
    case CONV_FIN: {
      const ConvForm f = route.form;
      ca.by = op.fin_by; ca.bx = op.fin_bx;
      ca.h2_oscale = op.h2_oscale;
      const bool ends = le && le->zo_end && op.ca.out == m->eps_cl;
      if (ends) { ca.zo_first = le->zo_first; ca.zo_end = le->zo_end; }
      CM_HIP(cm::launch_conv_fin(ca, f == FORM_F16 ? op.d_wfin16 : f == FORM_H2 ? op.d_wfin_h2 : op.d_wfin, f == FORM_F16 ? 1 : f == FORM_H2 ? 3 : f == FORM_B3 ? 2 : 0, st,
                                 ends && le->fuse ? le->step : nullptr, ends ? le->fuse : 0));
      break;
    }
    case CONV_SMALLN:
      CM_HIP(cm::launch_conv_smalln(ca, op.MB, op.d_wsmall, st));
      break;
    case CONV_1X1_F16:
      ca.wfrag = op.d_w1x1_16;
      CM_HIP(cm::launch_conv1x1_f16(ca, op.NB, st));
      break;
    case CONV_GENERIC:
      if (route.form == FORM_F16) { ca.wfrag = op.d_wfrag16; ca.wpar_stride = op.wpar_stride16; ca.f16 = 1; }
      CM_HIP(cm::launch_conv(ca, op.MB, op.NB, st));
      break;
  }
  return 0;
}

int run_ops(cm_model *m, const FwdPlan &plan, hipStream_t st, int b0 = 0, int slab = 0, const LoopEnds *le = nullptr) {
  const std::vector<Op> &ops = m->ops; const int B = plan.ctx.B;
  for (size_t oi = 0; oi < ops.size(); ++oi) {
    const Op &op = ops[oi]; const OpPlan &p = plan.ops[oi];
    if (!p.launch) continue;
    hipEvent_t e0 = nullptr, e1 = nullptr;
    if (m->profile) {
      CM_HIP(hipEventCreate(&e0));
      CM_HIP(hipEventCreate(&e1));
      CM_HIP(hipEventRecord(e0, st));
    }
    static const bool sync_ops = cm::diag_env("CM_SYNC_OPS") != nullptr;
    if (sync_ops) {
      const hipError_t e = hipDeviceSynchronize();
      fprintf(stderr, "[cm] forward reaches op %zu %s (%s)\n", oi, op.label.c_str(), hipGetErrorString(e));
      fflush(stderr);
    }
    switch (op.kind) {
      case OP_CONV:
        if (run_conv(m, op, plan, p, st, b0, slab, le)) return 1;
        break;
      case OP_STATS:
        CM_HIP(cm::launch_chan_stats(op.act->d + (size_t)b0 * op.act->V() * op.act->C, B, op.act->V(), op.act->C, p.ns_out,
                                     slot_part(op.act, p.ns_out, b0), slot_cnt(op.act, p.ns_out, b0), st));
        break;
      case OP_GNFIN:
        if (run_gnfin(op, p, B, st, b0)) return 1;
        break;
      case OP_ATTN: {
        const bool f16 = plan.ctx.precision == CM_PRECISION_F16 && !plan.ctx.train_fwd && op.E / ATTN_HEADS == 32 && !cm::diag_env("CM_NO_ATTN_F16");
        CM_HIP((f16 ? cm::launch_attn_core_f16 : cm::launch_attn_core)(op.qkv + (size_t)b0 * op.S * 3 * op.E, op.aout + (size_t)b0 * op.S * op.E,
                                                                      B, op.S, op.E, ATTN_HEADS, st));
        break;
      }
      case OP_ATTNBLK: {
        const Op &gop = ops[op.ab_gn], &qop = ops[op.ab_qkv], &oop = ops[op.ab_outc];
        float *scratch = m->ks_scratch + (size_t)slab * m->ks_scratch_floats;
        const size_t xoff = (size_t)b0 * op.S * op.E;
        cm::AttnBlockArgs aa{};
        aa.x = op.ab_x->d + xoff; aa.gamma = gop.gamma; aa.beta = gop.beta;
        aa.w_in = op.d_win; aa.b_in = qop.ca.bias; aa.w_out = op.d_wout;
        aa.part = scratch; aa.B = B; aa.S = op.S; aa.E = op.E; aa.heads = ATTN_HEADS; aa.groups = GN_GROUPS; aa.eps = GN_EPS;
        CM_HIP(cm::launch_attn_block(aa, st));
        cm::CombineArgs cb{};
        cb.part = scratch; cb.S = ATTN_HEADS; cb.stride = (long long)B * op.S * op.E;
        cb.bias = oop.ca.bias; cb.temb = nullptr; cb.tidx = m->tbuf;
        cb.resid = aa.x; cb.res_cs = op.E;
        cb.out = op.ab_out->d + xoff; cb.C = op.E; cb.V = op.S; cb.B = B;
        cb.nslots = p.ns_out; cb.stat_part = slot_part(op.ab_out, p.ns_out, b0); cb.stat_cnt = slot_cnt(op.ab_out, p.ns_out, b0);
        if (run_combine(cb, ops, plan, p.carries, b0, st)) return 1;
        break;
      }
    }
    if (m->profile) {
      CM_HIP(hipEventRecord(e1, st));
      m->prof_events[slab & 3].push_back({(int)oi, {e0, e1}});
    }
  }
  return 0;
}

int prof_begin(cm_model *m, hipStream_t st) {
  if (!m->profile) return 0;
  for (int i = 0; i < K_NCLASS; ++i) { m->prof_ms[i] = 0; m->prof_n[i] = 0; m->prof_union_ms[i] = 0; }
  for (Op &op : m->ops) { op.prof_ms = 0; op.prof_n = 0; }
  if (!m->prof_base) CM_HIP(hipEventCreate(&m->prof_base));
  CM_HIP(hipEventRecord(m->prof_base, st));
  return 0;
}

int prof_collect(cm_model *m, hipStream_t st) {
  if (!m->profile) return 0;
  CM_HIP(hipDeviceSynchronize()); (void)st;
  m->prof_B = m->plan.ctx.B;
  std::vector<std::pair<float, float>> iv[K_NCLASS];
  for (int ln = 0; ln < 4; ++ln) {
    for (auto &pe : m->prof_events[ln]) {
      float t0 = 0, t1 = 0;
      CM_HIP(hipEventElapsedTime(&t0, m->prof_base, pe.second.first));
      CM_HIP(hipEventElapsedTime(&t1, m->prof_base, pe.second.second));
      const float ms = t1 - t0;
      Op &op = m->ops[pe.first];
      op.prof_ms += ms;
      op.prof_n += 1;
      m->prof_ms[op.cls] += ms;
      m->prof_n[op.cls] += 1;
      iv[op.cls].push_back({t0, t1});
      hipEventDestroy(pe.second.first);
      hipEventDestroy(pe.second.second);
    }
    m->prof_events[ln].clear();
  }
  for (int c = 0; c < K_NCLASS; ++c) {
    std::sort(iv[c].begin(), iv[c].end());
    float total = 0, lo = 0, hi = -1;
    for (auto &x : iv[c]) {
      if (hi < lo || x.first > hi) { if (hi >= lo) total += hi - lo; lo = x.first; hi = x.second; }
      else hi = std::max(hi, x.second);
    }
    if (hi >= lo) total += hi - lo;
    m->prof_union_ms[c] = total;
  }
  return 0;
}

struct DevGuard {
  int prev = -1, cur = -1;
  explicit DevGuard(int dev) : cur(dev) {
    if (hipGetDevice(&prev) != hipSuccess) prev = -1;
    if (prev != dev) hipSetDevice(dev);
  }
  ~DevGuard() {
    if (prev >= 0 && prev != cur) hipSetDevice(prev);
  }
  DevGuard(const DevGuard &) = delete;
  DevGuard &operator=(const DevGuard &) = delete;
};

int check_ready(cm_model *m, int B) {
  if (!m) return fail("null model handle");
  if (!m->finalized) return fail("cm_model_finalize has not been called");
  if (B < 1 || B > m->cfg.max_batch) return fail("batch %d outside [1, max_batch=%d]", B, m->cfg.max_batch);
  return 0;
}

int make_plan(const cm_model *m, bool train_fwd, int B, FwdPlan *plan) {
  *plan = plan_forward(m->ops, FwdCtx{m->precision, train_fwd, m->h2_stale, B});
  return plan->err.empty() ? 0 : fail("%s", plan->err.c_str());
}

int plan_debug_conv(const cm_model *m, const Op &op, int index, int B, int src_slots, hipStream_t st, FwdPlan *plan) {
  if (!m->plan.err.empty() || m->plan.ops.size() != m->ops.size()) return fail("no forward has run on this handle");
  *plan = m->plan; plan->ctx = FwdCtx{m->precision, false, m->h2_stale, B};
  OpPlan &p = plan->ops[index], &gp = plan->ops[std::max(op.gn_op, 0)];
  p.carries = -1;
// ... 727 lines not shown
    } else if (op.kind == OP_ATTN) {
      f += 4.0 * op.S * (double)op.S * op.E * B;
    }
  }
  double wbytes = 0;
  for (const Param &p : m->params) wbytes += 4.0 * p.numel();
  if (flops) *flops = f;
  if (bytes) *bytes = by + wbytes;
  return 0;
}

int cm_profile_report(cm_model *m, char *buf, int64_t capacity) {
  CM_NOT_DIT(m, "cm_profile_report");
  if (!m || !buf || capacity < 1) return fail("null argument");
  std::string out;
  char line[512];
  for (const Op &op : m->ops) {
    if (op.prof_n == 0) continue;
    const double us = op.prof_ms * 1e3 / op.prof_n;
    if (op.kind == OP_CONV) {
      const cm::ConvArgs &a = op.ca;
      const double tf = op.flops_per_sample * m->prof_B / (us * 1e-6) / 1e12;
      snprintf(line, sizeof(line), "%-52s %9.1f us %7.2f TF %8.1f MF/sample B%d ks%d  %s%d NB%d box %dx%dx%dx%d grid %dx%d CK%d lds %zu\n", op.label.c_str(), us, tf,
               op.flops_per_sample / 1e6, m->prof_B, op.ks,
               "MB", op.MB, op.NB, a.bs, a.bz, a.by, a.bx, a.nts * a.ntz * a.nty * a.ntx,
               (a.Co + 32 * op.NB - 1) / (32 * op.NB), a.CK, cm::conv_lds_bytes(a, op.MB, op.NB));
    } else {
      snprintf(line, sizeof(line), "%-52s %9.1f us\n", op.label.c_str(), us);
    }
    out += line;
  }
  snprintf(buf, (size_t)capacity, "%s", out.c_str());
  return 0;
}

int cm_frame_metrics(int32_t device, const float *d_pred, const float *d_gt, int32_t N, int32_t Cc, int32_t H, int32_t W,
                     int32_t F, double *h_out, float *h_minmax) {
  if (!d_pred || !d_gt || !h_out || !h_minmax) return fail("null argument");
  if (N < 1 || Cc < 1 || H < 1 || W < 1 || F < 1) return fail("bad shape");
  DevGuard g(device);
  const size_t cells = (size_t)N * Cc * F;
  double *d_out = nullptr;
  float *d_mm = nullptr;
  CM_HIP(hipMalloc((void **)&d_out, cells * 8 * sizeof(double)));
  hipError_t e = hipMalloc((void **)&d_mm, cells * 2 * sizeof(float));
  if (e == hipSuccess) e = cm::launch_frame_metrics(d_pred, d_gt, N, Cc, H, W, F, d_out, d_mm, nullptr);
  if (e == hipSuccess) e = hipDeviceSynchronize();
  if (e == hipSuccess) e = hipMemcpy(h_out, d_out, cells * 8 * sizeof(double), hipMemcpyDeviceToHost);
  if (e == hipSuccess) e = hipMemcpy(h_minmax, d_mm, cells * 2 * sizeof(float), hipMemcpyDeviceToHost);
  hipFree(d_out);
  if (d_mm) hipFree(d_mm);
  if (e != hipSuccess) return fail("frame metrics failed: %s", hipGetErrorString(e));
  return 0;
}

int cm_mass_preservation_grad(int32_t device, const float *d_x, int32_t B, int32_t Cc, int32_t H, int32_t W, int32_t L,
                              float delta_t, float delta_l, float eps, float *d_grad, void *stream) {
  if (!d_x || !d_grad) return fail("null argument");
  if (B < 1 || H < 1 || W < 1 || L < 1) return fail("bad shape [%d,%d,%d,%d,%d]", B, Cc, H, W, L);
  if (Cc < 3) return fail("mass_preservation gradient needs >= 3 channels (r, u, v: guidance.py:25-31), got %d", Cc);
  if (delta_t == 0.f || delta_l == 0.f) return fail("delta_t and delta_l must be non-zero");
  if (d_x == d_grad) return fail("d_grad must not alias d_x (the gradient is written out of place)");
  DevGuard g(device);
  CM_HIP(cm::launch_mass_grad(d_x, Cc, d_grad, Cc, B, H, W, L, delta_t, delta_l, eps, (hipStream_t)stream));
  return 0;
}

int cm_debug_conv_flags(int32_t flags) {
  cm::conv_dbg_override = flags;
  return 0;
}

int cm_debug_conv_count(const cm_model *m, int32_t *count) {
  CM_NOT_DIT(m, "cm_debug_conv_count");
  if (!m || !m->finalized || !count) return fail("model not finalized");
  *count = (int32_t)m->ops.size();
  return 0;
}

int cm_debug_conv_info(const cm_model *m, int32_t index, char *buf, int64_t capacity) {
  CM_NOT_DIT(m, "cm_debug_conv_info");
  if (!m || !m->finalized || !buf || index < 0 || index >= (int)m->ops.size()) return fail("bad argument");
  const Op &op = m->ops[index];
  if (op.kind != OP_CONV) { snprintf(buf, (size_t)capacity, "other %s", op.label.c_str()); return 0; }
  const cm::ConvArgs &a = op.ca;
  const ConvRoute r = conv_route(op, m->precision, false, m->h2_stale);
  const LoopEnds le = loop_ends_plan(m->ops, m->x8, m->eps_cl, m->loop_ends, m->precision, m->h2_stale, m->cfg.past_len, m->cfg.future_len,
                                     m->cfg.in_channels, m->cfg.out_channels);
  char tail[64] = "";
  if (r.kernel == CONV_FIRST && a.src0 == m->x8) snprintf(tail, sizeof tail, " loop_ztiles %d/%d", le.tz_first, a.ntz);
  if (r.kernel == CONV_FIN && a.out == m->eps_cl && le.zo_end) snprintf(tail, sizeof tail, " loop_planes %d:%d fuse %d", le.zo_first, le.zo_end, le.fuse);
  snprintf(buf, (size_t)capacity, "conv %s %d %d %d %d %d %d %d %d %d %d %d %d %d %d %d %d %d %d %d %s %d%s", op.label.c_str(), a.ntaps, a.stride, a.par,
           a.C0 + a.C1, a.Co, a.Zo, a.Yo, a.Xo, op.NB, op.MB, a.bz, a.by, a.bx, op.ks,
           (op.small_n ? 1 : 0) | (op.first_k ? 2 : 0) | (op.stat_act ? 4 : 0) | (op.skip_if_fused ? 8 : 0) | (a.CK == 32 ? 16 : 0),
           op.out_act ? op.out_act->C : a.Co,
           a.C0, a.C1, op.wino ? 1 : 0,
           kConvKernelName[r.kernel], (int)r.form, tail);
  return 0;
}

extern "C" int cm_debug_loop_ends(cm_model *m, int32_t mask) {
  CM_NOT_DIT(m, "cm_debug_loop_ends");
  if (!m || mask < 0 || mask > 15) return fail("bad argument");
  m->loop_ends = mask;
  return 0;
}

int cm_debug_conv_io(cm_model *m, int32_t index, int32_t mode, const float *h_in0, const float *h_in1, float *h_out, int32_t B) {
  CM_NOT_DIT(m, "cm_debug_conv_io");
  if (check_ready(m, B)) return 1;
  if (!h_in0 || !h_out || index < 0 || index >= (int)m->ops.size()) return fail("bad argument");
  const Op &op = m->ops[index];
  if (op.kind != OP_CONV || !op.in0 || !op.out_act) return fail("op %d is not a convolution", index);
  if ((op.in1 != nullptr) != (h_in1 != nullptr)) return fail("op %d has %d source tensors", index, op.in1 ? 2 : 1);
  DevGuard g(m->device);
  hipStream_t st = m->stream;
  const size_t Vs = (size_t)op.in0->V(), Vo = (size_t)op.out_act->V();
  CM_HIP(hipMemcpy(op.in0->d, h_in0, (size_t)B * Vs * op.in0->C * sizeof(float), hipMemcpyHostToDevice));
  if (op.in1) CM_HIP(hipMemcpy(op.in1->d, h_in1, (size_t)B * Vs * op.in1->C * sizeof(float), hipMemcpyHostToDevice));
  if (mode < 0 || mode > 3) return fail("mode %d", mode);
  Op tmp = op;
  if (mode != 3) {
    tmp.ca.gn = nullptr; tmp.ca.silu = 0; tmp.ca.temb = nullptr; tmp.temb_off = -1; tmp.ca.resid = nullptr; tmp.resid_act = nullptr;
    tmp.d_s2w = nullptr; tmp.d_wqr_skip = nullptr; tmp.dbg_raw = true; tmp.pm_off = -1;
    if (!tmp.qr) tmp.gn_op = -1;
  }
  tmp.skip_if_fused = false;
  tmp.dbg_h2 = mode == 2;
  if (mode == 1) { tmp.d_wwino_b6 = nullptr; tmp.d_wqr_b6 = nullptr; tmp.d_wups_b6 = nullptr; }
  int src_slots = 0;
  if (mode == 2 && op.ups && op.in0->part) {
    const Act *t = op.in0;
    src_slots = t->nslice;
    CM_HIP(cm::launch_chan_stats(t->d, B, t->V(), t->C, src_slots, t->part, t->cnt, st));
  }
  FwdPlan plan;
  const int rc = plan_debug_conv(m, tmp, index, B, src_slots, st, &plan) || run_conv(m, tmp, plan, plan.ops[index], st, 0, 0);
  const hipError_t e = hipStreamSynchronize(st);
  if (rc) return 1;
  if (e != hipSuccess) return fail("debug conv launch failed: %s", hipGetErrorString(e));
  CM_HIP(hipMemcpy(h_out, op.out_act->d, (size_t)B * Vo * op.out_act->C * sizeof(float), hipMemcpyDeviceToHost));
  return 0;
}

int cm_debug_wino_form_counts(int64_t counts[16], int32_t reset) {
  if (!counts) return fail("bad argument");
  long long c[16];
  cm::conv_wino_form_counts(c, reset != 0);
  for (int i = 0; i < 16; ++i) counts[i] = (int64_t)c[i];
  return 0;
}

int cm_debug_conv_stats(cm_model *m, int32_t index, int32_t B, float *h_part, float *h_cnt, int32_t *nslots, int32_t *C) {
  CM_NOT_DIT(m, "cm_debug_conv_stats");
  if (check_ready(m, B)) return 1;
  if (!nslots || !C || index < 0 || index >= (int)m->ops.size()) return fail("bad argument");
  const Op &op = m->ops[index];
  if (op.kind != OP_CONV || !op.stat_act || !op.stat_act->part) return fail("op %d writes no statistics", index);
  const Act *t = op.stat_act;
  const int ns = (size_t)index < m->plan.ops.size() ? m->plan.ops[index].ns_out : 0;
  *nslots = ns; *C = t->C;
  DevGuard g(m->device);
  CM_HIP(hipStreamSynchronize(m->stream));
  if (h_part) CM_HIP(hipMemcpy(h_part, t->part, (size_t)B * ns * t->C * 2 * sizeof(float), hipMemcpyDeviceToHost));
  if (h_cnt) CM_HIP(hipMemcpy(h_cnt, t->cnt, (size_t)B * ns * sizeof(float), hipMemcpyDeviceToHost));
  return 0;
}

int cm_debug_time_conv(cm_model *m, int32_t index, int32_t MB, int32_t bz, int32_t by, int32_t bx, int32_t B,
                       int32_t iters, float *us) {
  CM_NOT_DIT(m, "cm_debug_time_conv");
  if (check_ready(m, B)) return 1;
  if (!us || index < 0 || index >= (int)m->ops.size() || iters < 1) return fail("bad argument");
  const Op &own = m->ops[index];
  if (own.kind != OP_CONV || ((own.first_k || own.wino) && MB > 0)) return fail("op %d is not a tunable convolution", index);
  DevGuard g(m->device);
  hipStream_t st = m->stream;
  Op op = own; op.skip_if_fused = false;
  int rc = 0;
  if (MB > 0) {
    cm::ConvArgs &a = op.ca;
    const int osd = a.par ? 2 : 1;
    if (bz < 1 || by < 1 || bx < 1 || (bz * by * bx + 31) / 32 != MB || !cm::conv_variant_exists(MB, op.NB)) rc = fail("invalid geometry");
    if (!rc) {
      a.bs = 1; a.bz = bz; a.by = by; a.bx = bx;
      op.MB = MB;
      a.ntz = (a.Zo / osd + bz - 1) / bz; a.nty = (a.Yo / osd + by - 1) / by; a.ntx = (a.Xo / osd + bx - 1) / bx;
      if (cm::conv_lds_bytes(a, MB, op.NB) > 80 * 1024) rc = fail("tile needs too much LDS");
      if (!rc && op.small_n && (MB & (MB - 1))) rc = fail("small-N kernel needs a power-of-two MB");
      if (!rc && cm::conv_halo_voxels(a) > 16384) rc = fail("halo box too large");
    }
    if (!rc) {
      std::vector<int> hv((size_t)cm::conv_halo_voxels(a)), mt((size_t)32 * MB);
      cm::conv_build_tables(a, MB, hv.data(), mt.data());
      hipError_t e = hipMemcpy(op.d_hvtab, hv.data(), hv.size() * sizeof(int), hipMemcpyHostToDevice);
      if (e == hipSuccess) e = hipMemcpy(op.d_mtab, mt.data(), mt.size() * sizeof(int), hipMemcpyHostToDevice);
      if (e != hipSuccess) rc = fail("table upload failed");
    }
  }
  FwdPlan plan;
  if (!rc) rc = plan_debug_conv(m, op, index, B, 0, st, &plan);
  if (!rc) {
    hipEvent_t e0 = nullptr, e1 = nullptr;
    hipEventCreate(&e0); hipEventCreate(&e1);
    for (int i = 0; i < 2 && !rc; ++i) rc = run_conv(m, op, plan, plan.ops[index], st, 0, 0);
    hipEventRecord(e0, st);
    for (int i = 0; i < iters && !rc; ++i) rc = run_conv(m, op, plan, plan.ops[index], st, 0, 0);
    hipEventRecord(e1, st);
    hipError_t e = hipStreamSynchronize(st);
    if (!rc && e != hipSuccess) rc = fail("timed launch failed: %s", hipGetErrorString(e));
    float ms = 0.f;
    if (!rc) { hipEventElapsedTime(&ms, e0, e1); *us = ms * 1e3f / (float)iters; }
    hipEventDestroy(e0); hipEventDestroy(e1);
  }
  if (MB > 0) {
    std::vector<int> hv((size_t)cm::conv_halo_voxels(own.ca)), mt((size_t)32 * own.MB);
    cm::conv_build_tables(own.ca, own.MB, hv.data(), mt.data());
    CM_HIP(hipMemcpy(own.d_hvtab, hv.data(), hv.size() * sizeof(int), hipMemcpyHostToDevice));
    CM_HIP(hipMemcpy(own.d_mtab, mt.data(), mt.size() * sizeof(int), hipMemcpyHostToDevice));
  }
  return rc;
}

static int exec_flops_split(const cm_model *m, int32_t B, double flops[8], double *b16) {
  CM_NOT_DIT(m, "the exec / issue FLOP split");
  if (!m || !m->finalized || !flops) return fail("model not finalized");
  for (int i = 0; i < 8; ++i) flops[i] = 0;
  if (b16) for (int i = 0; i < 8; ++i) b16[i] = 0;
  for (const Op &op : m->ops) {
    if (op.kind == OP_ATTN) { flops[op.cls] += 4.0 * op.S * (double)op.S * op.E * B; continue; }
    if (op.kind != OP_CONV) continue;
    const ConvRoute r = conv_route(op, m->precision, false, m->h2_stale);
    double mult16 = r.form == FORM_F16 ? 1.0 : r.form == FORM_B6 ? 6.0 : r.form == FORM_FP32 ? 0.0 : 3.0;
    const cm::ConvArgs &a = op.ca;
    const double Ci = a.C0 + a.C1, Cskip = op.skip0 ? op.skip0->C + (op.skip1 ? op.skip1->C : 0) : 0;
    double f = op.flops_per_sample;
    switch (r.kernel) {
      case CONV_NONE: continue;
      case CONV_F16D:
        f = (double)(a.Zo / op.f16d_bz) * (a.Yo / op.f16d_by) * (a.Xo / op.f16d_bx) * 128.0 * op.f16d_mbw * a.Co * (Ci * 27.0 + Cskip) * 2;
        break;
      case CONV_FIN:
        f = (double)(a.Yo / op.fin_by) * (a.Xo / op.fin_bx) * a.Zo * 64.0 * 128.0 * 32.0 * 2;
        break;
      case CONV_QR:
        f = 2.0 * (a.Yo * a.Xo > 32 ? 2 : 1) * 32 * a.Co * (Ci * 18.0 + Cskip) * 2;
        break;
      case CONV_WINO:
        f = (double)a.ntz * a.nty * a.ntx * ((a.Co + 31) / 32) * (16.0 * 32 * 32 * Ci * 3 * 2 + 4.0 * 32 * 32 * Cskip * 2);
        break;
      case CONV_UPS: {
        const double tiles = (double)(a.Zs / op.ups_tz) * (a.Ys / op.ups_ty) * (a.Xs / op.ups_tx);
        const double pairs = 2.0 * op.ups_mbw - ((op.ups_planes && op.ups_tz == a.Zs) ? 1.0 : 0.0);
        f = tiles * 8.0 * 32.0 * pairs * 4.0 * a.Co * Ci * 2;
        break;
      }
      case CONV_1X1_F16: mult16 = 0.0;
      default:
        if (a.par) f = f * 8.0 / 27.0;
        if (cm::conv_zsplit_variant(a, op.MB, op.NB)) f *= a.par ? 6.0 / 8.0 : 18.0 / 27.0;
    }
    if (b16 && mult16 > 0.0) b16[op.cls] += mult16 * f * B;
    else flops[op.cls] += f * B;
  }
  return 0;
}

int cm_model_exec_flops(const cm_model *m, int32_t B, double flops[8]) { return exec_flops_split(m, B, flops, nullptr); }

int cm_model_issue_flops(const cm_model *m, int32_t B, double f32[8], double b16[8]) {
  if (!b16) return fail("null output");
  return exec_flops_split(m, B, f32, b16);
}

int cm_model_class_flops(const cm_model *m, int32_t B, double flops[8]) {
  CM_NOT_DIT(m, "cm_model_class_flops");
  if (!m || !m->finalized || !flops) return fail("model not finalized");
  for (int i = 0; i < 8; ++i) flops[i] = 0;
  for (const Op &op : m->ops) {
    if (op.kind == OP_CONV) flops[op.cls] += op.flops_per_sample * B;
    else if (op.kind == OP_ATTN) flops[op.cls] += 4.0 * op.S * (double)op.S * op.E * B;
  }
  return 0;
}

}

#include "cm_train_host.inc"
```

### crowdmod-ddpm-4d_amd/csrc/cm_train_host.inc

```

struct cm_train_state {
  std::set<const Act *> gset;
  size_t nfloats = 0;
  std::map<std::string, size_t> poff;
  float *pbuf = nullptr, *gbuf = nullptr, *mbuf = nullptr, *vbuf = nullptr;
  float lr = 5e-5f, b1 = 0.5f, b2 = 0.999f, eps = 1e-8f, wd = 0.003f;
  float dropout = 0.1f;
  int step = 0;
  hipEvent_t ev_dy = nullptr, ev_wdone = nullptr;
  struct Derived { float *dst; int *d_idx; float *d_coef; int nk; long long n; bool bwd_only; };
  std::vector<Derived> derived;
  cm::PackJob *d_jobs = nullptr;
  int *d_blk2job = nullptr; long long pack_blocks = 0;
  struct DerivedWino { float *dst; int *d_idx27; int Co, Ci, Ci_pad; long long n; };
  std::vector<DerivedWino> derived_wino;
  cm::WinoPackJob *d_wjobs = nullptr; int *d_wblk2job = nullptr; long long wpack_blocks = 0;
  int njobs = 0;
  long long pack_total = 0;
  struct Dgrad {
    bool have = false;
    cm::ConvArgs ca{};
    int MB = 1, NB = 1;
    int *d_hv = nullptr, *d_mt = nullptr;
    float *wfrag = nullptr, *zero_bias = nullptr;
// ... 55 lines not shown
    }
  return out;
}

std::vector<int> pack_conv_indices(const std::vector<int> &src, int nk, int Co, int Ci, int ntaps, int Ci_pad, int CK, int NB) {
  const int TN = 32 * NB, ntn = (Co + TN - 1) / TN, nch = Ci_pad / CK, K8 = CK / 8, nsteps = ntaps * K8;
  std::vector<int> out((size_t)ntn * nch * nsteps * NB * 64 * 4 * nk, -1);
  size_t o = 0;
  for (int nt = 0; nt < ntn; ++nt)
    for (int ch = 0; ch < nch; ++ch)
      for (int s = 0; s < nsteps; ++s) {
        const int t = s / K8, j = s % K8;
        for (int nb = 0; nb < NB; ++nb)
          for (int lane = 0; lane < 64; ++lane)
            for (int jj = 0; jj < 4; ++jj, ++o) {
              const int co = nt * TN + nb * 32 + (lane & 31);
              const int ci = ch * CK + 8 * j + 4 * (lane >> 5) + jj;
              if (co < Co && ci < Ci)
                for (int k = 0; k < nk; ++k) out[o * nk + k] = src[(((size_t)co * Ci + ci) * ntaps + t) * nk + k];
            }
      }
  return out;
}

int add_derived(cm_model *m, float *dst, const std::vector<int> &idx, int nk, bool bwd_only = false,
                const std::vector<float> *coef = nullptr) {
  cm_train_state::Derived d;
  d.dst = dst; d.nk = nk; d.n = (long long)(idx.size() / nk); d.bwd_only = bwd_only; d.d_coef = nullptr;
  if (dev_alloc(m, (void **)&d.d_idx, idx.size() * sizeof(int))) return 1;
  CM_HIP(hipMemcpy(d.d_idx, idx.data(), idx.size() * sizeof(int), hipMemcpyHostToDevice));
  if (coef) {
    if (coef->size() != idx.size()) return fail("derived tensor: coefficient / index size mismatch");
    if (dev_alloc(m, (void **)&d.d_coef, coef->size() * sizeof(float))) return 1;
    CM_HIP(hipMemcpy(d.d_coef, coef->data(), coef->size() * sizeof(float), hipMemcpyHostToDevice));
  }
  m->train->derived.push_back(d);
  return 0;
}

int add_derived_wino(cm_model *m, float *dst, const std::vector<int> &idx27, int Co, int Ci, int Ci_pad) {
  cm_train_state::DerivedWino d;
  d.dst = dst; d.Co = Co; d.Ci = Ci; d.Ci_pad = Ci_pad;
  d.n = (long long)((Co + 31) / 32) * 32 * Ci_pad * 3;
  if ((long long)idx27.size() != (long long)Co * Ci * 27) return fail("Winograd weight map: %zu indices for %d x %d x 27", idx27.size(), Co, Ci);
  if (dev_alloc(m, (void **)&d.d_idx27, idx27.size() * sizeof(int))) return 1;
  CM_HIP(hipMemcpy(d.d_idx27, idx27.data(), idx27.size() * sizeof(int), hipMemcpyHostToDevice));
  m->train->derived_wino.push_back(d);
  return 0;
}

int tune_launch(cm_model *m, cm::ConvArgs &ca, int &MB, int NB, int *&d_hv, int *&d_mt, bool wgrad) {
  Op tmp;
  tmp.kind = OP_CONV; tmp.ca = ca; tmp.NB = NB;
  static Act dummy;
  tmp.stat_act = wgrad ? &dummy : nullptr;
  if (wgrad) tmp.ca.CK = 32;
  pick_tile(tmp, TUNE_BATCH);
  const int ck = ca.CK;
  ca = tmp.ca; ca.CK = ck; MB = tmp.MB;
  std::vector<int> hv((size_t)cm::conv_halo_voxels(ca)), mt((size_t)32 * MB);
  cm::conv_build_tables(ca, MB, hv.data(), mt.data());
  if (dev_alloc(m, (void **)&d_hv, hv.size() * sizeof(int))) return 1;
  if (dev_alloc(m, (void **)&d_mt, mt.size() * sizeof(int))) return 1;
  CM_HIP(hipMemcpy(d_hv, hv.data(), hv.size() * sizeof(int), hipMemcpyHostToDevice));
  CM_HIP(hipMemcpy(d_mt, mt.data(), mt.size() * sizeof(int), hipMemcpyHostToDevice));
  ca.hvtab = d_hv; ca.mtab = d_mt;
  return 0;
}

int refresh_h2(cm_model *m) {
  if (!m->h2_stale) return 0;
  cm_train_state *T = m->train;
  if (!T || m->precision != CM_PRECISION_F32) { m->h2_stale = false; return 0; }
  DevGuard g(m->device);
  CM_HIP(hipDeviceSynchronize());
  auto fetch = [&](const std::string &name, std::vector<float> *out) -> int {
    const Param &pr = P(m, name);
    out->resize((size_t)pr.numel());
    CM_HIP(hipMemcpy(out->data(), T->pbuf + T->poff[name], out->size() * sizeof(float), hipMemcpyDeviceToHost));
    return 0;
  };
  std::vector<float> w, gam, bet, frag;
  for (Op &op : m->ops) {
    if (op.kind != OP_CONV || !(op.d_wwino_h2 || op.d_wqr_h2 || op.d_wfin_h2 || op.d_wups_h2)) continue;
    const int Co = op.ca.Co, Ci = op.ca.C0 + op.ca.C1;
    if (fetch(op.wname, &w)) return 1;
    op.h2_off = false;
    if (!op.d_wups_h2) {
      if (op.gn_op < 0) { op.h2_off = true; continue; }
      const Op &gop = m->ops[op.gn_op];
      if (fetch(gop.gname, &gam) || fetch(gop.bename, &bet)) return 1;
      if (!h2_bound_ok(gam, bet, gop, op.d_wwino_h2 ? 4.0 : 1.0)) { op.h2_off = true; continue; }
    }
    float ws = 0.f;
    float *dst = nullptr;
    if (op.d_wfin_h2) {
      ws = h2_wscale(w.data(), w.size());
      if (ws > 0.f) CM_HIP(cm::launch_fin_pack(T->pbuf + T->poff[op.wname], op.d_wfin_h2, Co, 2, m->stream, ws));
    } else if (op.d_wwino_h2) {
      ws = h2_pack_wino(w.data(), Co, Ci, Ci, &frag); dst = op.d_wwino_h2;
    } else if (op.d_wqr_h2) {
      ws = h2_pack_qr(w.data(), Co, Ci, &frag); dst = op.d_wqr_h2;
    } else {
      ws = h2_pack_ups(w.data(), Co, Ci, &frag); dst = op.d_wups_h2;
    }
    if (!(ws > 0.f)) { op.h2_off = true; continue; }
    if (dst) CM_HIP(hipMemcpy(dst, frag.data(), frag.size() * sizeof(float), hipMemcpyHostToDevice));
    op.h2_oscale = 1.f / ws;
  }
  CM_HIP(hipStreamSynchronize(m->stream));
  m->h2_stale = false;
  return 0;
}

int repack_all(cm_model *m, hipStream_t st) {
  cm_train_state *T = m->train;
  m->h2_stale = true;
  if (!T->d_jobs) {
    std::vector<cm::PackJob> jobs;
    std::vector<int> b2j;
    long long total = 0;
    for (auto &d : T->derived) {
      cm::PackJob j{};
      j.dst = d.dst; j.idx = d.d_idx; j.coef = d.d_coef; j.start = total; j.nk = d.nk;
      j.n = d.n; j.blk0 = (long long)b2j.size();
      for (long long k = 0; k < (d.n + 255) / 256; ++k) b2j.push_back((int)jobs.size());
      jobs.push_back(j);
      total += d.n;
    }
    if (dev_alloc(m, (void **)&T->d_jobs, jobs.size() * sizeof(cm::PackJob))) return 1;
    if (dev_alloc(m, (void **)&T->d_blk2job, b2j.size() * sizeof(int))) return 1;
    CM_HIP(hipMemcpy(T->d_jobs, jobs.data(), jobs.size() * sizeof(cm::PackJob), hipMemcpyHostToDevice));
    CM_HIP(hipMemcpy(T->d_blk2job, b2j.data(), b2j.size() * sizeof(int), hipMemcpyHostToDevice));
    T->njobs = (int)jobs.size();
    T->pack_total = total;
    T->pack_blocks = (long long)b2j.size();
  }
  CM_HIP(cm::launch_gather_pack_jobs(T->pbuf, T->d_jobs, T->d_blk2job, T->pack_blocks, st));
  if (!T->d_wjobs && !T->derived_wino.empty()) {
    std::vector<cm::WinoPackJob> jobs;
    std::vector<int> b2j;
    for (auto &d : T->derived_wino) {
      cm::WinoPackJob j{};
      j.dst = d.dst; j.idx27 = d.d_idx27; j.Co = d.Co; j.Ci = d.Ci; j.Ci_pad = d.Ci_pad; j.n = d.n; j.blk0 = (long long)b2j.size();
      for (long long k = 0; k < (d.n + 255) / 256; ++k) b2j.push_back((int)jobs.size());
      jobs.push_back(j);
    }
    if (dev_alloc(m, (void **)&T->d_wjobs, jobs.size() * sizeof(cm::WinoPackJob))) return 1;
    if (dev_alloc(m, (void **)&T->d_wblk2job, b2j.size() * sizeof(int))) return 1;
    CM_HIP(hipMemcpy(T->d_wjobs, jobs.data(), jobs.size() * sizeof(cm::WinoPackJob), hipMemcpyHostToDevice));
    CM_HIP(hipMemcpy(T->d_wblk2job, b2j.data(), b2j.size() * sizeof(int), hipMemcpyHostToDevice));
    T->wpack_blocks = (long long)b2j.size();
  }
  CM_HIP(cm::launch_wino_pack_jobs(T->pbuf, T->d_wjobs, T->d_wblk2job, T->wpack_blocks, st));
  for (Op &op : m->ops) {
    if (op.kind != OP_CONV) continue;
    if (op.d_wups_b6)
      CM_HIP(cm::launch_ups_b6_repack(op.ca.wfrag, op.ca.wpar_stride, op.d_wups_b6, op.wups_b6_stride, op.ca.Co, op.ca.C0, op.NB, st));
    if (op.d_wwino_b6) CM_HIP(cm::launch_wino_b6_repack(op.d_wwino, op.d_wwino_b6, op.wwino_floats, st));
    if (op.d_wqr_b6) CM_HIP(cm::launch_qr_b6_repack(op.d_wqr, op.d_wqr_b6, op.wqr_floats, op.ca.C0 + op.ca.C1, st));
    if (op.d_wfin) CM_HIP(cm::launch_fin_pack(T->pbuf + T->poff[op.wname], op.d_wfin, op.ca.Co, 0, st));
  }
  for (auto &D : T->dg) {
    if (D.wwino_b6) CM_HIP(cm::launch_wino_b6_repack(D.wwino, D.wwino_b6, D.wwino_floats, st));
    if (D.qr) CM_HIP(cm::launch_qr_b6_repack(D.wqr, D.wqr_b6, D.wqr_floats, D.ca.C0, st));
  }
// ... 759 lines not shown
```

### crowdmod-ddpm-4d_amd/native.py

```python
from __future__ import annotations

import ctypes as C
import importlib.util
import os
from typing import Optional

import numpy as np

_HERE = os.path.dirname(os.path.abspath(__file__))
LIB_PATH = os.environ.get("CM_LIB_PATH") or os.path.join(_HERE, "libcrowdmod_hip.so")
MAX_LEVELS = 8
ABI_VERSION = 3


class NativeError(RuntimeError):
    """A libcrowdmod_hip call returned non-zero (message from cm_last_error)."""


class cm_unet_config(C.Structure):
    _fields_ = [
        ("in_channels", C.c_int32), ("out_channels", C.c_int32), ("num_res_blocks", C.c_int32),
        ("base_channels", C.c_int32), ("n_levels", C.c_int32),
        ("channel_mult", C.c_int32 * MAX_LEVELS), ("apply_attention", C.c_int32 * MAX_LEVELS),
        ("time_multiple", C.c_int32), ("rows", C.c_int32), ("cols", C.c_int32),
# ... 63 lines not shown
    "cm_unet_forward_train": (C.c_int, [_P, _P, _P, _P, _P, C.c_float, C.c_uint64, C.c_int64, _P, C.c_int32, _P]),
    "cm_mse_loss": (C.c_int, [_P, _P, _P, C.c_int64, C.POINTER(C.c_float), _P]),
    "cm_debug_activation": (C.c_int, [_P, C.c_char_p, _P, C.c_int64, C.POINTER(C.c_int64)]),
    "cm_schedule_create": (C.c_int, [C.c_int32, C.c_float, C.c_float, C.c_float, C.c_int32, C.POINTER(_P)]),
    "cm_schedule_destroy": (C.c_int, [_P]),
    "cm_schedule_table": (C.c_int, [_P, C.c_int32, _P, C.c_int32]),
    "cm_q_sample": (C.c_int, [_P, _P, _P, _P, _P, C.c_int32, C.c_int64, _P]),
    "cm_ddpm_step": (C.c_int, [_P, _P, _P, C.c_int32, _P, C.c_uint64, C.c_int64, C.c_int32, C.c_int64, _P]),
    "cm_sample_loop": (C.c_int, [_P, _P, _P, _P, _P, C.POINTER(cm_sample_opts), _P, _P, C.c_int32, _P]),
    "cm_sample_loop_host": (C.c_int, [_P, _P, _P, _P, _P, C.POINTER(cm_sample_opts), _P, _P, C.c_int32]),
    "cm_sample_num_steps": (C.c_int, [_P, C.POINTER(cm_sample_opts), C.POINTER(C.c_int32)]),
    "cm_profile_enable": (C.c_int, [_P, C.c_int32]),
    "cm_profile_read": (C.c_int, [_P, _F, C.POINTER(C.c_int64)]),
    "cm_profile_read_union": (C.c_int, [_P, _F]),
    "cm_profile_report": (C.c_int, [_P, C.c_char_p, C.c_int64]),
    "cm_model_cost": (C.c_int, [_P, C.c_int32, C.POINTER(C.c_double), C.POINTER(C.c_double)]),
    "cm_model_class_flops": (C.c_int, [_P, C.c_int32, C.POINTER(C.c_double)]),
    "cm_model_exec_flops": (C.c_int, [_P, C.c_int32, C.POINTER(C.c_double)]),
    "cm_model_issue_flops": (C.c_int, [_P, C.c_int32, C.POINTER(C.c_double), C.POINTER(C.c_double)]),
    "cm_frame_metrics": (C.c_int, [C.c_int32, _P, _P, C.c_int32, C.c_int32, C.c_int32, C.c_int32, C.c_int32, _P, _P]),
    "cm_mass_preservation_grad": (C.c_int, [C.c_int32, _P, C.c_int32, C.c_int32, C.c_int32, C.c_int32, C.c_int32,
                                            C.c_float, C.c_float, C.c_float, _P, _P]),
    "cm_debug_conv_flags": (C.c_int, [C.c_int32]),
    "cm_debug_conv_count": (C.c_int, [_P, C.POINTER(C.c_int32)]),
    "cm_debug_conv_info": (C.c_int, [_P, C.c_int32, C.c_char_p, C.c_int64]),
    "cm_debug_conv_io": (C.c_int, [_P, C.c_int32, C.c_int32, _P, _P, _P, C.c_int32]),
    "cm_debug_conv_stats": (C.c_int, [_P, C.c_int32, C.c_int32, _P, _P, _P, _P]),
    "cm_debug_wino_form_counts": (C.c_int, [_P, C.c_int32]),
    "cm_debug_time_conv": (C.c_int, [_P, C.c_int32, C.c_int32, C.c_int32, C.c_int32, C.c_int32, C.c_int32, C.c_int32,
                                     C.POINTER(C.c_float)]),
    "cm_train_init": (C.c_int, [_P, C.c_float, C.c_float, C.c_float, C.c_float, C.c_float, C.c_float]),
    "cm_train_set_lr": (C.c_int, [_P, C.c_float]),
    "cm_train_set_sample_base": (C.c_int, [_P, C.c_int64]),
    "cm_train_step": (C.c_int, [_P, _P, _P, _P, _P, _P, _P, C.c_uint64, C.POINTER(C.c_float), C.c_int32, C.c_int32, _P]),
    "cm_train_step_xt": (C.c_int, [_P, _P, _P, _P, _P, _P, C.c_uint64, C.POINTER(C.c_float), C.c_int32, C.c_int32, _P]),
    "cm_train_get_grad": (C.c_int, [_P, C.c_char_p, _P, C.c_int64]),
    "cm_train_sync": (C.c_int, [_P]),
    "cm_train_flat_grads": (C.c_int, [_P, C.POINTER(_P), C.POINTER(C.c_int64)]),
    "cm_train_apply": (C.c_int, [_P, _P]),
    "cm_train_get_opt_state": (C.c_int, [_P, C.c_char_p, C.c_int32, _P, C.c_int64]),
    "cm_train_set_opt_state": (C.c_int, [_P, C.c_char_p, C.c_int32, _P, C.c_int64]),
    "cm_train_opt_step": (C.c_int, [_P, C.POINTER(C.c_int32), C.c_int32]),
}


def _preload_hip_runtime():
    spec = importlib.util.find_spec("torch")
    if spec is None or not spec.submodule_search_locations:
        return
    cand = os.path.join(list(spec.submodule_search_locations)[0], "lib", "libamdhip64.so")
    if os.path.exists(cand):
        try:
            C.CDLL(cand, mode=C.RTLD_GLOBAL)
        except OSError:
            pass


def lib() -> C.CDLL:
    global _lib
    if _lib is not None:
        return _lib
    if not os.path.exists(LIB_PATH):
        raise NativeError(
            f"{LIB_PATH} is missing: build it with `python -c 'import __graft_entry__ as g; g.build()'` "
            "(or `make -C crowdmod-ddpm-4d_amd/csrc`). There is no CPU fallback.")
    _preload_hip_runtime()
    L = C.CDLL(LIB_PATH)
    for name, (res, args) in SIGNATURES.items():
        fn = getattr(L, name)
        fn.restype = res
        fn.argtypes = args
    if L.cm_abi_version() != ABI_VERSION:
        raise NativeError("libcrowdmod_hip.so ABI version mismatch")
    _lib = L
    return L


def check(rc: int) -> None:
    if rc != 0:
        msg = lib().cm_last_error()
        raise NativeError(msg.decode("utf-8", "replace") if msg else f"libcrowdmod_hip call failed ({rc})")


def device_count() -> int:
    n = C.c_int(0)
    check(lib().cm_device_count(C.byref(n)))
    return n.value


def ptr(x) -> int:
    if x is None:
        return None
    if isinstance(x, int):
        return x
    if isinstance(x, np.ndarray):
        return x.ctypes.data
    if isinstance(x, DeviceBuffer):
        return x.ptr
    if hasattr(x, "data_ptr"):
        return x.data_ptr()
    raise TypeError(f"cannot take the address of {type(x)}")


class DeviceBuffer:

    def __init__(self, nbytes: int, device: int = 0):
        self.device, self.nbytes = device, int(nbytes)
        p = C.c_void_p()
        check(lib().cm_malloc(device, C.byref(p), self.nbytes))
        self.ptr = p.value

    def upload(self, arr: np.ndarray) -> "DeviceBuffer":
        arr = np.ascontiguousarray(arr)
        assert arr.nbytes <= self.nbytes
        check(lib().cm_memcpy_h2d(self.device, self.ptr, arr.ctypes.data, arr.nbytes))
        return self

    def download(self, shape, dtype=np.float32) -> np.ndarray:
        out = np.empty(shape, dtype=dtype)
        assert out.nbytes <= self.nbytes
        check(lib().cm_memcpy_d2h(self.device, out.ctypes.data, self.ptr, out.nbytes))
        return out

    @classmethod
    def from_array(cls, arr: np.ndarray, device: int = 0) -> "DeviceBuffer":
        arr = np.ascontiguousarray(arr)
        return cls(arr.nbytes, device).upload(arr)

    def free(self):
        if getattr(self, "ptr", None):
            lib().cm_free(self.device, self.ptr)
            self.ptr = None

    def __del__(self):
        try:
            self.free()
        except Exception:
            pass
```

Before: 936.3 denoise-steps/s, aggregate over 1 GPU under weak scaling (every GPU advances its own batch of 64 chains per step).

## Add whole-sample fused attention kernel with f16 split-product MFMA projections

```diff
diff --git a/crowdmod-ddpm-4d_amd/csrc/cm_attn_block.hip b/crowdmod-ddpm-4d_amd/csrc/cm_attn_block.hip
--- a/crowdmod-ddpm-4d_amd/csrc/cm_attn_block.hip
+++ b/crowdmod-ddpm-4d_amd/csrc/cm_attn_block.hip
@@ -1,6 +1,7 @@
 #include "cm_kernels.h"
 
 #include <algorithm>
+#include <atomic>
 
 namespace cm {
 
@@ -300,4 +301,304 @@
   return hipErrorInvalidValue;
 }
 
-}
+
+typedef _Float16 f16x8a __attribute__((ext_vector_type(8)));
+typedef unsigned u32x4a __attribute__((ext_vector_type(4)));
+
+constexpr int AS_NT = 1024, AS_E = 128, AS_D = 32, AS_SMAX = 64;
+constexpr int AS_HS = AS_E + 8;
+constexpr int AS_QS = AS_E + 4;
+constexpr int AS_RED = 512;
+
+size_t attn_sample_lds_bytes() {
+  return (size_t)2 * AS_SMAX * AS_HS * sizeof(_Float16) + ((size_t)3 * AS_SMAX * AS_QS + AS_RED) * sizeof(float);
+}
+
+bool attn_sample_ok(int S, int E, int heads, int groups) { return E == AS_E && heads == 4 && groups == 8 && S >= 1 && S <= AS_SMAX; }
+
+__device__ __forceinline__ float as_range_scale(float m, float *inv) {
+  const unsigned e = (__float_as_uint(m) >> 23) & 255u;
+  int se = 267 - (int)e;
+  se = se < 32 ? 32 : (se > 222 ? 222 : se);
+  if (!(m > 0.f) || e == 255u) se = 127;
+  *inv = __uint_as_float((unsigned)(254 - se) << 23);
+  return __uint_as_float((unsigned)se << 23);
+}
+
+__global__ __launch_bounds__(AS_NT) void attn_sample_kernel(const AttnSampleArgs a) {
+  constexpr int E = AS_E, D = AS_D, HS = AS_HS, QS = AS_QS, NT = AS_NT;
+  extern __shared__ __attribute__((aligned(16))) unsigned char smraw[];
+  _Float16 *XH = reinterpret_cast<_Float16 *>(smraw);
+  _Float16 *XM = XH + AS_SMAX * HS;
+  float *Qs = reinterpret_cast<float *>(XM + AS_SMAX * HS);
+  float *Ks = Qs + AS_SMAX * QS;
+  float *Vs = Ks + AS_SMAX * QS;
+  float *red = Vs + AS_SMAX * QS;
+  const int S = a.S, b = blockIdx.x, tid = threadIdx.x;
+  const int lane = tid & 63, wave = __builtin_amdgcn_readfirstlane(tid >> 6);
+  const int r16 = lane & 15, g4 = lane >> 4;
+  const int nrb = (S + 15) >> 4;
+
+  const int q4 = tid & 31, rl = tid >> 5;
+  const float *xb = a.x + (size_t)b * S * E;
+  f32x4 vx[2];
+#pragma unroll
+  for (int u = 0; u < 2; ++u) vx[u] = *reinterpret_cast<const f32x4 *>(xb + (size_t)min(rl + 32 * u, S - 1) * E + 4 * q4);
+  const f32x4 ga = *reinterpret_cast<const f32x4 *>(a.gamma + 4 * q4);
+  const f32x4 be = *reinterpret_cast<const f32x4 *>(a.beta + 4 * q4);
+  const int cb0 = 3 * (wave >> 1), rbp = wave & 1;
+  const u32x4a *wing = reinterpret_cast<const u32x4a *>(a.win_h2);
+  u32x4a wf[3][4][2];
+  float bias[3];
+#pragma unroll
+  for (int ci = 0; ci < 2; ++ci) {
+#pragma unroll
+    for (int ks = 0; ks < 4; ++ks)
+#pragma unroll
+      for (int t = 0; t < 2; ++t) wf[ci][ks][t] = wing[(((size_t)(cb0 + ci) * 4 + ks) * 2 + t) * 64 + lane];
+  }
+#pragma unroll
+  for (int ci = 0; ci < 3; ++ci) bias[ci] = a.b_in[(cb0 + ci) * 16 + r16];
+
+  const int grp = q4 >> 2;
+  auto group_sum = [&](float v, float *slot) -> float {
+    v += __shfl_xor(v, 1);
+    v += __shfl_xor(v, 2);
+    v += __shfl_xor(v, 32);
+    if ((lane & 35) == 0) slot[wave * 8 + grp] = v;
+    __syncthreads();
+    float t = 0.f;
+#pragma unroll
+    for (int w = 0; w < NT / 64; ++w) t += slot[w * 8 + grp];
+    return t;
+  };
+  float s1 = 0.f;
+#pragma unroll
+  for (int u = 0; u < 2; ++u)
+    if (rl + 32 * u < S) s1 += (vx[u][0] + vx[u][1]) + (vx[u][2] + vx[u][3]);
+  const float cnt = (float)(E / 8) * (float)S;
+  const float mean = group_sum(s1, red) / cnt;
+  float s2 = 0.f;
+#pragma unroll
+  for (int u = 0; u < 2; ++u)
+    if (rl + 32 * u < S) {
+      const float d0 = vx[u][0] - mean, d1 = vx[u][1] - mean, d2 = vx[u][2] - mean, d3 = vx[u][3] - mean;
+      s2 += (d0 * d0 + d1 * d1) + (d2 * d2 + d3 * d3);
+    }
+  const float rstd = rsqrtf(group_sum(s2, red + 128) / cnt + a.eps);
+
+  f32x4 xn[2];
+  float amax = 0.f;
+  {
+    const f32x4 sc = ga * rstd;
+    const f32x4 sh = be - sc * mean;
+#pragma unroll
+    for (int u = 0; u < 2; ++u) {
+      xn[u] = vx[u] * sc + sh;
+      if (rl + 32 * u < S) amax = fmaxf(amax, fmaxf(fmaxf(fabsf(xn[u][0]), fabsf(xn[u][1])), fmaxf(fabsf(xn[u][2]), fabsf(xn[u][3]))));
+      else xn[u] = f32x4{0.f, 0.f, 0.f, 0.f};
+    }
+  }
+  auto sample_max = [&](float v, float *slot) -> float {
+#pragma unroll
+    for (int off = 32; off >= 1; off >>= 1) v = fmaxf(v, __shfl_xor(v, off));
+    if (lane == 0) slot[wave] = v;
+    __syncthreads();
+    float m = slot[0];
+#pragma unroll
+    for (int w = 1; w < NT / 64; ++w) m = fmaxf(m, slot[w]);
+    return m;
+  };
+  float isa;
+  const float sa = as_range_scale(sample_max(amax, red + 272), &isa);
+#pragma unroll
+  for (int u = 0; u < 2; ++u) {
+    cm_u32x2_t t3[3];
+    cm_split2_f16(xn[u] * sa, t3);
+    const int row = rl + 32 * u;
+    *reinterpret_cast<cm_u32x2_t *>(XH + row * HS + 4 * q4) = t3[0];
+    *reinterpret_cast<cm_u32x2_t *>(XM + row * HS + 4 * q4) = t3[1];
+  }
+  __syncthreads();
+
+  {
+    const float osc = a.in_oscale * isa, qscale = rsqrtf((float)D);
+#pragma unroll
+    for (int ci = 0; ci < 3; ++ci) {
+      const int cb = cb0 + ci;
+      const int which = cb >> 3, c = (cb & 7) * 16 + r16;
+      float *dst = which == 0 ? Qs : (which == 1 ? Ks : Vs);
+      for (int rb = rbp; rb < nrb; rb += 2) {
+        const _Float16 *ah = XH + (rb * 16 + r16) * HS + 8 * g4, *am = XM + (rb * 16 + r16) * HS + 8 * g4;
+        f32x4 acc = {0.f, 0.f, 0.f, 0.f};
+#pragma unroll
+        for (int ks = 0; ks < 4; ++ks) {
+          const f16x8a xh = *reinterpret_cast<const f16x8a *>(ah + 32 * ks), xm = *reinterpret_cast<const f16x8a *>(am + 32 * ks);
+          const f16x8a wh = __builtin_bit_cast(f16x8a, wf[ci][ks][0]), wm = __builtin_bit_cast(f16x8a, wf[ci][ks][1]);
+          acc = __builtin_amdgcn_mfma_f32_16x16x32_f16(xh, wm, acc, 0, 0, 0);
+          acc = __builtin_amdgcn_mfma_f32_16x16x32_f16(xm, wh, acc, 0, 0, 0);
+          acc = __builtin_amdgcn_mfma_f32_16x16x32_f16(xh, wh, acc, 0, 0, 0);
+        }
+#pragma unroll
+        for (int reg = 0; reg < 4; ++reg) {
+          float v = acc[reg] * osc + bias[ci];
+          if (which == 0) v *= qscale;
+          dst[(rb * 16 + 4 * g4 + reg) * QS + c] = v;
+        }
+      }
+      if (ci == 0) {
+#pragma unroll
+        for (int ks = 0; ks < 4; ++ks)
+#pragma unroll
+          for (int t = 0; t < 2; ++t) wf[2][ks][t] = wing[(((size_t)(cb0 + 2) * 4 + ks) * 2 + t) * 64 + lane];
+      }
+    }
+  }
+  const u32x4a *woutg = reinterpret_cast<const u32x4a *>(a.wout_h2);
+  const f32x4 bo = *reinterpret_cast<const f32x4 *>(a.b_out + 4 * q4);
+#pragma unroll
+  for (int u = 0; u < 2; ++u)
+    vx[u] = *reinterpret_cast<const f32x4 *>(xb + (size_t)min(rl + 32 * u, S - 1) * E + 4 * q4);
+#pragma unroll
+  for (int ks = 0; ks < 4; ++ks)
+#pragma unroll
+    for (int t = 0; t < 2; ++t) wf[0][ks][t] = woutg[(((size_t)(wave >> 1) * 4 + ks) * 2 + t) * 64 + lane];
+  __syncthreads();
+
+  const int h = wave >> 2, qb = wave & 3;
+  f32x4 oT[2] = {{0.f, 0.f, 0.f, 0.f}, {0.f, 0.f, 0.f, 0.f}};
+  float omax = 0.f;
+  const bool qvalid = qb * 16 + r16 < S;
+  if (qb < nrb) {
+    const float *qp = Qs + (qb * 16 + r16) * QS + h * D + 8 * g4;
+    const f32x4 q0 = *reinterpret_cast<const f32x4 *>(qp), q1 = *reinterpret_cast<const f32x4 *>(qp + 4);
+    f32x4 sc[4];
+    float mx = -3.0e38f;
+#pragma unroll
+    for (int kb = 0; kb < 4; ++kb) {
+      sc[kb] = f32x4{-3.0e38f, -3.0e38f, -3.0e38f, -3.0e38f};
+      if (kb < nrb) {
+        const float *kp = Ks + (kb * 16 + r16) * QS + h * D + 8 * g4;
+        const f32x4 k0 = *reinterpret_cast<const f32x4 *>(kp), k1 = *reinterpret_cast<const f32x4 *>(kp + 4);
+        f32x4 acc = {0.f, 0.f, 0.f, 0.f};
+#pragma unroll
+        for (int j = 0; j < 4; ++j) acc = __builtin_amdgcn_mfma_f32_16x16x4f32(k0[j], q0[j], acc, 0, 0, 0);
+#pragma unroll
+        for (int j = 0; j < 4; ++j) acc = __builtin_amdgcn_mfma_f32_16x16x4f32(k1[j], q1[j], acc, 0, 0, 0);
+#pragma unroll
+        for (int reg = 0; reg < 4; ++reg) {
+          sc[kb][reg] = (kb * 16 + 4 * g4 + reg < S) ? acc[reg] : -3.0e38f;
+          mx = fmaxf(mx, sc[kb][reg]);
+        }
+      }
+    }
+    mx = fmaxf(mx, __shfl_xor(mx, 16));
+    mx = fmaxf(mx, __shfl_xor(mx, 32));
+    float l = 0.f;
+#pragma unroll
+    for (int kb = 0; kb < 4; ++kb)
+#pragma unroll
+      for (int reg = 0; reg < 4; ++reg) {
+        const float p = (kb < nrb && kb * 16 + 4 * g4 + reg < S) ? __expf(sc[kb][reg] - mx) : 0.f;
+        sc[kb][reg] = p;
+        l += p;
+      }
+    l += __shfl_xor(l, 16);
+    l += __shfl_xor(l, 32);
+#pragma unroll
+    for (int kb = 0; kb < 4; ++kb)
+      if (kb < nrb) {
+#pragma unroll
+        for (int reg = 0; reg < 4; ++reg) {
+          const float *vp = Vs + (kb * 16 + 4 * g4 + reg) * QS + h * D + r16;
+          oT[0] = __builtin_amdgcn_mfma_f32_16x16x4f32(vp[0], sc[kb][reg], oT[0], 0, 0, 0);
+          oT[1] = __builtin_amdgcn_mfma_f32_16x16x4f32(vp[16], sc[kb][reg], oT[1], 0, 0, 0);
+        }
+      }
+    const float inv = 1.0f / l;
+    oT[0] *= inv;
+    oT[1] *= inv;
+    if (qvalid) {
+#pragma unroll
+      for (int db = 0; db < 2; ++db)
+        omax = fmaxf(omax, fmaxf(fmaxf(fabsf(oT[db][0]), fabsf(oT[db][1])), fmaxf(fabsf(oT[db][2]), fabsf(oT[db][3]))));
+    }
+  }
+  float iso;
+  const float so = as_range_scale(sample_max(omax, red + 288), &iso);
+  if (qb < nrb) {
+#pragma unroll
+    for (int db = 0; db < 2; ++db) {
+      cm_u32x2_t t3[3];
+      cm_split2_f16(qvalid ? oT[db] * so : f32x4{0.f, 0.f, 0.f, 0.f}, t3);
+      const int off = (qb * 16 + r16) * HS + h * D + 16 * db + 4 * g4;
+      *reinterpret_cast<cm_u32x2_t *>(XH + off) = t3[0];
+      *reinterpret_cast<cm_u32x2_t *>(XM + off) = t3[1];
+    }
+  }
+  __syncthreads();
+
+  {
+    const float osc = a.out_oscale * iso;
+    const int c = (wave >> 1) * 16 + r16;
+    for (int rb = rbp; rb < nrb; rb += 2) {
+      const _Float16 *ah = XH + (rb * 16 + r16) * HS + 8 * g4, *am = XM + (rb * 16 + r16) * HS + 8 * g4;
+      f32x4 acc = {0.f, 0.f, 0.f, 0.f};
+#pragma unroll
+      for (int ks = 0; ks < 4; ++ks) {
+        const f16x8a xh = *reinterpret_cast<const f16x8a *>(ah + 32 * ks), xm = *reinterpret_cast<const f16x8a *>(am + 32 * ks);
+        const f16x8a wh = __builtin_bit_cast(f16x8a, wf[0][ks][0]), wm = __builtin_bit_cast(f16x8a, wf[0][ks][1]);
+        acc = __builtin_amdgcn_mfma_f32_16x16x32_f16(xh, wm, acc, 0, 0, 0);
+        acc = __builtin_amdgcn_mfma_f32_16x16x32_f16(xm, wh, acc, 0, 0, 0);
+        acc = __builtin_amdgcn_mfma_f32_16x16x32_f16(xh, wh, acc, 0, 0, 0);
+      }
+#pragma unroll
+      for (int reg = 0; reg < 4; ++reg) Qs[(rb * 16 + 4 * g4 + reg) * QS + c] = acc[reg] * osc;
+    }
+  }
+  __syncthreads();
+
+  float *ob = a.out + (size_t)b * S * E;
+#pragma unroll
+  for (int u = 0; u < 2; ++u) {
+    const int row = rl + 32 * u;
+    if (row < S) {
+      f32x4 *yp = reinterpret_cast<f32x4 *>(Qs + row * QS + 4 * q4);
+      const f32x4 y = (*yp + bo) + vx[u];
+      *yp = y;
+      *reinterpret_cast<f32x4 *>(ob + (size_t)row * E + 4 * q4) = y;
+    }
+  }
+  if (!a.stat_part) return;
+  __syncthreads();
+  if (tid < E * a.nslots) {
+    const int c = tid & (E - 1), slot = tid >> 7;
+    const int r0 = slot * 32, r1 = min(S, r0 + 32);
+    float tot = 0.f;
+    for (int r = r0; r < r1; ++r) tot += Qs[r * QS + c];
+    const float n = (float)(r1 - r0);
+    const float mu = tot / n;
+    float m2 = 0.f;
+    for (int r = r0; r < r1; ++r) { const float d = Qs[r * QS + c] - mu; m2 += d * d; }
+    float *sp = a.stat_part + (((size_t)b * a.nslots + slot) * E + c) * 2;
+    sp[0] = mu;
+    sp[1] = m2;
+    if (c == 0) a.stat_cnt[(size_t)b * a.nslots + slot] = n;
+  }
+}
+
+hipError_t launch_attn_sample(const AttnSampleArgs &a, hipStream_t st) {
+  if (!attn_sample_ok(a.S, AS_E, 4, 8) || a.B < 1 || a.nslots != (a.S + 31) / 32 || !a.win_h2 || !a.wout_h2) return hipErrorInvalidValue;
+  static std::atomic<bool> attr_set[64];
+  int dev = 0;
+  (void)hipGetDevice(&dev);
+  if (!attr_set[dev & 63].load(std::memory_order_acquire)) {
+    hipError_t e = hipFuncSetAttribute(reinterpret_cast<const void *>(attn_sample_kernel), hipFuncAttributeMaxDynamicSharedMemorySize, 160 * 1024);
+    if (e != hipSuccess) return e;
+    attr_set[dev & 63].store(true, std::memory_order_release);
+  }
+  hipLaunchKernelGGL(attn_sample_kernel, dim3(a.B), dim3(AS_NT), attn_sample_lds_bytes(), st, a);
+  return hipGetLastError();
+}
+
+}
diff --git a/crowdmod-ddpm-4d_amd/csrc/cm_attn_plan_selftest.cpp b/crowdmod-ddpm-4d_amd/csrc/cm_attn_plan_selftest.cpp
--- /dev/null
+++ b/crowdmod-ddpm-4d_amd/csrc/cm_attn_plan_selftest.cpp
@@ -0,0 +1,138 @@
+#include "cm_model.cpp"
+
+#include <cstdio>
+#include <memory>
+
+namespace {
+
+int failures = 0;
+#define EXPECT(cond)                                                                  \
+  do {                                                                                \
+    if (!(cond)) { fprintf(stderr, "%s:%d: EXPECT(%s) failed\n", __FILE__, __LINE__, #cond); ++failures; } \
+  } while (0)
+
+struct List {
+  std::vector<std::unique_ptr<Act>> acts;
+  std::vector<Op> ops;
+  Act *act(int C, int Z, int Y, int X) {
+    static float buf[4];
+    acts.push_back(std::make_unique<Act>());
+    Act *a = acts.back().get();
+    a->C = C; a->Z = Z; a->Y = Y; a->X = X; a->part = a->cnt = buf;
+    return a;
+  }
+};
+
+List block_list(int Y, int X, bool frags, bool qr, bool with_fin = true) {
+  static float frag[4];
+  List L;
+  Act *x = L.act(128, 2, Y, X), *o = L.act(128, 2, Y, X);
+  Op fb;
+  fb.kind = OP_ATTNBLK; fb.cls = K_ATTN; fb.label = "attention (fused block)";
+  fb.ab_x = x; fb.ab_out = o; fb.S = 2 * Y * X; fb.E = 128;
+  if (frags) { fb.d_win_h2 = fb.d_wout_h2 = frag; fb.ab_in_oscale = fb.ab_out_oscale = 0.25f; }
+  L.ops.push_back(fb);
+  if (with_fin) {
+    Op g;
+    g.kind = OP_GNFIN; g.cls = K_NORM; g.g0 = o; g.label = "gn"; g.qr_consumer = qr;
+    L.ops.push_back(g);
+  }
+  return L;
+}
+
+FwdCtx ctx_of(int precision, bool train, bool stale = false, int B = 2) {
+  FwdCtx c;
+  c.precision = precision; c.train_fwd = train; c.h2_stale = stale; c.B = B;
+  return c;
+}
+
+void test_attention_plan() {
+  const int plans[4] = {CM_PRECISION_F32, CM_PRECISION_F32X, CM_PRECISION_F32R, CM_PRECISION_F16};
+  int cases = 0;
+  for (int prec : plans) {
+    {
+      const List L = block_list(3, 9, true, true);
+      const FwdPlan P = plan_forward(L.ops, ctx_of(prec, false));
+      EXPECT(P.err.empty() && P.ops[0].launch && P.ops[0].ns_out == 2 && P.ops[0].carries == -1);
+      EXPECT(P.ops[0].attn_sample == (prec == CM_PRECISION_F32));
+      EXPECT(P.ops[1].fin == FIN_QR && !P.ops[1].launch && P.ops[1].ns0 == 2);
+      EXPECT(plan_forward(L.ops, ctx_of(prec, false, false, 64)).ops[0].attn_sample == (prec == CM_PRECISION_F32));
+      ++cases;
+    }
+    {
+      const List L = block_list(3, 9, true, true, false);
+      const FwdPlan P = plan_forward(L.ops, ctx_of(prec, true));
+      EXPECT(P.err.empty() && !P.ops[0].launch && !P.ops[0].attn_sample && P.ops[0].ns_out == 0 && P.ops[0].carries == -1);
+      ++cases;
+    }
+    {
+      const List L = block_list(3, 9, true, false);
+      const FwdPlan P = plan_forward(L.ops, ctx_of(prec, false));
+      EXPECT(P.err.empty() && P.ops[0].launch && P.ops[0].carries == 1 && !P.ops[0].attn_sample && P.ops[0].ns_out == 2);
+      EXPECT(P.ops[1].fin == FIN_COMBINE && !P.ops[1].launch && P.ops[1].ns0 == 2);
+      ++cases;
+    }
+  }
+  {
+    const List L = block_list(3, 9, true, true);
+    const FwdPlan P = plan_forward(L.ops, ctx_of(CM_PRECISION_F32, false, true));
+    EXPECT(P.err.empty() && P.ops[0].launch && !P.ops[0].attn_sample && P.ops[0].ns_out == 2 && P.ops[1].fin == FIN_QR);
+    ++cases;
+  }
+  {
+    List L = block_list(3, 9, false, true);
+    EXPECT(!plan_forward(L.ops, ctx_of(CM_PRECISION_F32, false)).ops[0].attn_sample);
+    L = block_list(3, 9, true, true);
+    L.ops[0].ab_out_oscale = 0.f;
+    EXPECT(!plan_forward(L.ops, ctx_of(CM_PRECISION_F32, false)).ops[0].attn_sample);
+    L.ops[0].ab_out_oscale = 0.25f; L.ops[0].ab_in_oscale = 0.f;
+    EXPECT(!plan_forward(L.ops, ctx_of(CM_PRECISION_F32, false)).ops[0].attn_sample);
+    cases += 3;
+  }
+  {
+    struct T { int Y, X, S, ns; bool taken; };
+    const T tok[] = {{1, 1, 2, 1, true}, {4, 4, 32, 1, true}, {1, 17, 34, 2, true}, {4, 8, 64, 2, true}, {1, 33, 66, 3, false}, {3, 14, 84, 3, false}};
+    for (const T &t : tok) {
+      const List L = block_list(t.Y, t.X, true, true);
+      const FwdPlan P = plan_forward(L.ops, ctx_of(CM_PRECISION_F32, false));
+      EXPECT(L.ops[0].S == t.S && P.err.empty() && P.ops[0].launch && P.ops[0].ns_out == t.ns && P.ops[1].ns0 == t.ns);
+      EXPECT(P.ops[0].attn_sample == t.taken && cm::attn_sample_ok(t.S, 128, ATTN_HEADS, GN_GROUPS) == t.taken);
+      ++cases;
+    }
+    EXPECT(!cm::attn_sample_ok(0, 128, ATTN_HEADS, GN_GROUPS) && !cm::attn_sample_ok(65, 128, ATTN_HEADS, GN_GROUPS));
+    EXPECT(!cm::attn_sample_ok(54, 64, ATTN_HEADS, GN_GROUPS) && !cm::attn_sample_ok(54, 128, 8, GN_GROUPS) && !cm::attn_sample_ok(54, 128, ATTN_HEADS, 4));
+    EXPECT(cm::attn_sample_lds_bytes() <= 160 * 1024);
+  }
+  {
+    cm::AttnSampleArgs a{};
+    a.B = 2; a.S = 66; a.nslots = 3;
+    EXPECT(cm::launch_attn_sample(a, nullptr) == hipErrorInvalidValue);
+    a.S = 54; a.nslots = 2;
+    EXPECT(cm::launch_attn_sample(a, nullptr) == hipErrorInvalidValue);
+    ++cases;
+  }
+  {
+    std::vector<float> w((size_t)32 * 64);
+    for (size_t i = 0; i < w.size(); ++i) w[i] = (float)((int)(i % 97) - 48) * 0.0131f;
+    const float ws = h2_wscale(w.data(), w.size());
+    const std::vector<float> f = pack_attn_h2(w.data(), 32, 64, ws);
+    EXPECT(f.size() == (size_t)32 * 64);
+    const uint16_t *h = reinterpret_cast<const uint16_t *>(f.data());
+    const int n = 21, k = 45, cb = n / 16, ks = k / 32, lane = 16 * ((k % 32) / 8) + n % 16, i = k % 8;
+    const float hi = f16_bits_to_f32(h[((((size_t)cb * 2 + ks) * 2 + 0) * 64 + lane) * 8 + i]);
+    const float mid = f16_bits_to_f32(h[((((size_t)cb * 2 + ks) * 2 + 1) * 64 + lane) * 8 + i]);
+    const float v = w[(size_t)n * 64 + k] * ws;
+    EXPECT(std::fabs(hi + mid - v) <= std::ldexp(std::fabs(v), -21));
+    ++cases;
+  }
+  printf("test_attention_plan: %d cases\n", cases);
+}
+
+}
+
+int main() {
+  test_attention_plan();
+  if (failures) { fprintf(stderr, "%d failure(s)\n", failures); return 1; }
+  printf("attention plan selftest ok\n");
+  return 0;
+}
diff --git a/crowdmod-ddpm-4d_amd/csrc/cm_kernels.h b/crowdmod-ddpm-4d_amd/csrc/cm_kernels.h
--- a/crowdmod-ddpm-4d_amd/csrc/cm_kernels.h
+++ b/crowdmod-ddpm-4d_amd/csrc/cm_kernels.h
@@ -319,6 +319,21 @@
 size_t attn_block_lds_bytes(int S, int E, int heads);
 hipError_t launch_attn_block(const AttnBlockArgs &a, hipStream_t st);
 
+struct AttnSampleArgs {
+  const float *x;
+  const float *gamma, *beta;
+  const float *win_h2, *b_in;
+  const float *wout_h2, *b_out;
+  float in_oscale, out_oscale;
+  float *out;
+  float *stat_part, *stat_cnt;
+  int B, S, nslots;
+  float eps;
+};
+bool attn_sample_ok(int S, int E, int heads, int groups);
+size_t attn_sample_lds_bytes();
+hipError_t launch_attn_sample(const AttnSampleArgs &a, hipStream_t st);
+
 enum { DIT_PRO_NONE = 0, DIT_PRO_LN = 1, DIT_PRO_PATCH = 2 };
 enum { DIT_EPI_BIAS = 0, DIT_EPI_SILU = 1, DIT_EPI_SILU2 = 2, DIT_EPI_GELU = 3, DIT_EPI_GATE = 4, DIT_EPI_PATCH = 5,
        DIT_EPI_UNPATCH = 6 };
diff --git a/crowdmod-ddpm-4d_amd/csrc/cm_model.cpp b/crowdmod-ddpm-4d_amd/csrc/cm_model.cpp
--- a/crowdmod-ddpm-4d_amd/csrc/cm_model.cpp
+++ b/crowdmod-ddpm-4d_amd/csrc/cm_model.cpp
@@ -153,6 +153,8 @@
   int ab_gn = -1, ab_qkv = -1, ab_outc = -1;
   float *d_win = nullptr, *d_wout = nullptr;
   std::string win_name, wout_name;
+  float *d_win_h2 = nullptr, *d_wout_h2 = nullptr;
+  float ab_in_oscale = 0.f, ab_out_oscale = 0.f;
 };
 
 enum ConvKernel { CONV_NONE, CONV_QR, CONV_KSPLIT, CONV_UPS, CONV_F16D, CONV_WINO, CONV_FIRST, CONV_FIN, CONV_SMALLN, CONV_1X1_F16, CONV_GENERIC };
@@ -169,6 +171,7 @@
   int ns0 = 0, ns1 = 0;
   FinBy fin = FIN_NONE;
   int carries = -1;
+  bool attn_sample = false;
 };
 struct FwdPlan { FwdCtx ctx; std::vector<OpPlan> ops; std::string err; };
 
@@ -485,6 +488,23 @@
     out[t] = f32_to_bf16_bits(rem);
     rem -= bf16_bits_to_f32(out[t]);
   }
+}
+
+std::vector<float> pack_attn_h2(const float *W, int N, int K, float scale) {
+  const int ncb = N / 16, nks = K / 32;
+  std::vector<uint16_t> out((size_t)ncb * nks * 2 * 64 * 8, 0);
+  for (int cb = 0; cb < ncb; ++cb)
+    for (int ks = 0; ks < nks; ++ks)
+      for (int lane = 0; lane < 64; ++lane)
+        for (int i = 0; i < 8; ++i) {
+          const int n = cb * 16 + (lane & 15), k = ks * 32 + 8 * (lane >> 4) + i;
+          uint16_t t3[3];
+          f16_split2(W[(size_t)n * K + k], scale, t3);
+          for (int tm = 0; tm < 2; ++tm) out[(((((size_t)cb * nks + ks) * 2 + tm) * 64) + lane) * 8 + i] = t3[tm];
+        }
+  std::vector<float> packed(out.size() / 2);
+  std::memcpy(packed.data(), out.data(), out.size() * 2);
+  return packed;
 }
 
 std::vector<float> pack_ups_b6(const float *W, int Co, int Ci, float h2_scale = 0.f) {
@@ -867,6 +887,15 @@
     }
   }
   return ws;
+}
+
+static void attn_pack_h2(const float *w_in, const float *w_out, int E, std::vector<float> *f_in, std::vector<float> *f_out, float *osc_in,
+                         float *osc_out) {
+  const float wsi = h2_wscale(w_in, (size_t)3 * E * E), wso = h2_wscale(w_out, (size_t)E * E);
+  *f_in = pack_attn_h2(w_in, 3 * E, E, wsi);
+  *f_out = pack_attn_h2(w_out, E, E, wso);
+  *osc_in = wsi > 0.f ? 1.f / wsi : 0.f;
+  *osc_out = wso > 0.f ? 1.f / wso : 0.f;
 }
 
 int add_conv(cm_model *m, const ConvSpec &s) {
@@ -1260,6 +1289,11 @@
         fb.win_name = ap + ".mhsa.in_proj_weight"; fb.wout_name = ap + ".mhsa.out_proj.weight";
         if (upload(m, P(m, fb.win_name).host, &fb.d_win)) return 1;
         if (upload(m, P(m, fb.wout_name).host, &fb.d_wout)) return 1;
+        if (m->precision == CM_PRECISION_F32 && !cm::diag_env("CM_NO_H2") && cm::attn_sample_ok(fb.S, fb.E, ATTN_HEADS, GN_GROUPS)) {
+          std::vector<float> fi, fo;
+          attn_pack_h2(P(m, fb.win_name).host.data(), P(m, fb.wout_name).host.data(), fb.E, &fi, &fo, &fb.ab_in_oscale, &fb.ab_out_oscale);
+          if (upload(m, fi, &fb.d_win_h2) || upload(m, fo, &fb.d_wout_h2)) return 1;
+        }
         for (int i = nops - 4; i < nops; ++i) m->ops[i].in_attn_block = true;
         const size_t need = (size_t)ATTN_HEADS * m->cfg.max_batch * fb.S * fb.E;
         m->ks_scratch_floats = std::max(m->ks_scratch_floats, need);
@@ -1492,6 +1526,12 @@
   cm::ConvArgs a = c.ca;
   a.B = B; a.f16 = r.form == FORM_F16 ? a.f16 : (int)r.form;
   return r.kernel == CONV_WINO && r.form != FORM_FP32 && a.gn && cm::conv_wino_p_taken(a, r.form == FORM_F16, true);
+}
+
+bool attn_sample_planned(const Op &op, const FwdCtx &ctx) {
+  static const bool off = cm::diag_env("CM_NO_ATTN_SAMPLE") != nullptr;
+  return !off && !ctx.train_fwd && ctx.precision == CM_PRECISION_F32 && !ctx.h2_stale && op.d_win_h2 && op.d_wout_h2 &&
+         op.ab_in_oscale > 0.f && op.ab_out_oscale > 0.f && cm::attn_sample_ok(op.S, op.E, ATTN_HEADS, GN_GROUPS);
 }
 
 FwdPlan plan_forward(const std::vector<Op> &ops, const FwdCtx &ctx) {
@@ -1526,12 +1566,15 @@
     }
     int j = i + 1;
     while (j < n && !in_ctx(ops[j])) ++j;
-    if (!two_pass || no_fuse || j == n || ops[j].kind != OP_GNFIN || ops[j].g0 != two_pass || (ops[j].qr_consumer && infer)) continue;
-    const Act *g1 = ops[j].g1;
-    cm::CombineArgs cb{};
-    cb.C = pc; cb.V = pv; cb.B = ctx.B; cb.nslots = p.ns_out; cb.stat_part = two_pass->part; cb.fin_C1 = g1 ? g1->C : 0; cb.fin_groups = GN_GROUPS;
-    if ((g1 && (g1->V() != pv || slots_of(g1) < 1)) || !cm::combine_gn_ok(cb)) continue;
-    p.carries = j; P.ops[j].fin = FIN_COMBINE; P.ops[j].ns0 = p.ns_out; P.ops[j].ns1 = g1 ? slots_of(g1) : 0;
+    if (two_pass && !no_fuse && j < n && ops[j].kind == OP_GNFIN && ops[j].g0 == two_pass && !(ops[j].qr_consumer && infer)) {
+      const Act *g1 = ops[j].g1;
+      cm::CombineArgs cb{};
+      cb.C = pc; cb.V = pv; cb.B = ctx.B; cb.nslots = p.ns_out; cb.stat_part = two_pass->part; cb.fin_C1 = g1 ? g1->C : 0; cb.fin_groups = GN_GROUPS;
+      if (!(g1 && (g1->V() != pv || slots_of(g1) < 1)) && cm::combine_gn_ok(cb)) {
+        p.carries = j; P.ops[j].fin = FIN_COMBINE; P.ops[j].ns0 = p.ns_out; P.ops[j].ns1 = g1 ? slots_of(g1) : 0;
+      }
+    }
+    if (op.kind == OP_ATTNBLK) p.attn_sample = attn_sample_planned(op, ctx) && p.carries < 0;
   }
   return P;
 }
@@ -1740,6 +1783,35 @@
   return 0;
 }
 
+int run_attn_block(const cm_model *m, const Op &op, const FwdPlan &plan, const OpPlan &p, hipStream_t st, int b0, int slab) {
+  const std::vector<Op> &ops = m->ops; const int B = plan.ctx.B;
+  const Op &gop = ops[op.ab_gn], &qop = ops[op.ab_qkv], &oop = ops[op.ab_outc];
+  const size_t xoff = (size_t)b0 * op.S * op.E;
+  if (p.attn_sample) {
+    cm::AttnSampleArgs as{};
+    as.x = op.ab_x->d + xoff; as.gamma = gop.gamma; as.beta = gop.beta;
+    as.win_h2 = op.d_win_h2; as.b_in = qop.ca.bias; as.wout_h2 = op.d_wout_h2; as.b_out = oop.ca.bias;
+    as.in_oscale = op.ab_in_oscale; as.out_oscale = op.ab_out_oscale;
+    as.out = op.ab_out->d + xoff; as.B = B; as.S = op.S; as.nslots = p.ns_out; as.eps = GN_EPS;
+    as.stat_part = slot_part(op.ab_out, p.ns_out, b0); as.stat_cnt = slot_cnt(op.ab_out, p.ns_out, b0);
+    CM_HIP(cm::launch_attn_sample(as, st));
+    return 0;
+  }
+  float *scratch = m->ks_scratch + (size_t)slab * m->ks_scratch_floats;
+  cm::AttnBlockArgs aa{};
+  aa.x = op.ab_x->d + xoff; aa.gamma = gop.gamma; aa.beta = gop.beta;
+  aa.w_in = op.d_win; aa.b_in = qop.ca.bias; aa.w_out = op.d_wout;
+  aa.part = scratch; aa.B = B; aa.S = op.S; aa.E = op.E; aa.heads = ATTN_HEADS; aa.groups = GN_GROUPS; aa.eps = GN_EPS;
+  CM_HIP(cm::launch_attn_block(aa, st));
+  cm::CombineArgs cb{};
+  cb.part = scratch; cb.S = ATTN_HEADS; cb.stride = (long long)B * op.S * op.E;
+  cb.bias = oop.ca.bias; cb.temb = nullptr; cb.tidx = m->tbuf;
+  cb.resid = aa.x; cb.res_cs = op.E;
+  cb.out = op.ab_out->d + xoff; cb.C = op.E; cb.V = op.S; cb.B = B;
+  cb.nslots = p.ns_out; cb.stat_part = slot_part(op.ab_out, p.ns_out, b0); cb.stat_cnt = slot_cnt(op.ab_out, p.ns_out, b0);
+  return run_combine(cb, ops, plan, p.carries, b0, st);
+}
+
 int run_ops(cm_model *m, const FwdPlan &plan, hipStream_t st, int b0 = 0, int slab = 0, const LoopEnds *le = nullptr) {
   const std::vector<Op> &ops = m->ops; const int B = plan.ctx.B;
   for (size_t oi = 0; oi < ops.size(); ++oi) {
@@ -1774,24 +1846,9 @@
                                                                       B, op.S, op.E, ATTN_HEADS, st));
         break;
       }
-      case OP_ATTNBLK: {
-        const Op &gop = ops[op.ab_gn], &qop = ops[op.ab_qkv], &oop = ops[op.ab_outc];
-        float *scratch = m->ks_scratch + (size_t)slab * m->ks_scratch_floats;
-        const size_t xoff = (size_t)b0 * op.S * op.E;
-        cm::AttnBlockArgs aa{};
-        aa.x = op.ab_x->d + xoff; aa.gamma = gop.gamma; aa.beta = gop.beta;
-        aa.w_in = op.d_win; aa.b_in = qop.ca.bias; aa.w_out = op.d_wout;
-        aa.part = scratch; aa.B = B; aa.S = op.S; aa.E = op.E; aa.heads = ATTN_HEADS; aa.groups = GN_GROUPS; aa.eps = GN_EPS;
-        CM_HIP(cm::launch_attn_block(aa, st));
-        cm::CombineArgs cb{};
-        cb.part = scratch; cb.S = ATTN_HEADS; cb.stride = (long long)B * op.S * op.E;
-        cb.bias = oop.ca.bias; cb.temb = nullptr; cb.tidx = m->tbuf;
-        cb.resid = aa.x; cb.res_cs = op.E;
-        cb.out = op.ab_out->d + xoff; cb.C = op.E; cb.V = op.S; cb.B = B;
-        cb.nslots = p.ns_out; cb.stat_part = slot_part(op.ab_out, p.ns_out, b0); cb.stat_cnt = slot_cnt(op.ab_out, p.ns_out, b0);
-        if (run_combine(cb, ops, plan, p.carries, b0, st)) return 1;
+      case OP_ATTNBLK:
+        if (run_attn_block(m, op, plan, p, st, b0, slab)) return 1;
         break;
-      }
     }
     if (m->profile) {
       CM_HIP(hipEventRecord(e1, st));
@@ -2685,6 +2742,11 @@
   CM_NOT_DIT(m, "cm_debug_conv_info");
   if (!m || !m->finalized || !buf || index < 0 || index >= (int)m->ops.size()) return fail("bad argument");
   const Op &op = m->ops[index];
+  if (op.kind == OP_ATTNBLK) {
+    const FwdPlan pl = plan_forward(m->ops, FwdCtx{m->precision, false, m->h2_stale, m->plan.ctx.B});
+    snprintf(buf, (size_t)capacity, "other %s %s", op.label.c_str(), pl.ops[index].attn_sample ? "attn_sample_kernel" : "attn_head_kernel");
+    return 0;
+  }
   if (op.kind != OP_CONV) { snprintf(buf, (size_t)capacity, "other %s", op.label.c_str()); return 0; }
   const cm::ConvArgs &a = op.ca;
   const ConvRoute r = conv_route(op, m->precision, false, m->h2_stale);
@@ -2708,6 +2770,43 @@
   m->loop_ends = mask;
   return 0;
 }
+
+extern "C" int cm_debug_attn_block(cm_model *m, int32_t index, int32_t mode, const float *h_x, float *h_out, float *h_part, float *h_cnt,
+                                   int32_t B) {
+  CM_NOT_DIT(m, "cm_debug_attn_block");
+  if (check_ready(m, B)) return 1;
+  if (!h_x || !h_out || index < 0 || index >= (int)m->ops.size() || mode < 0 || mode > 1) return fail("bad argument");
+  const Op &op = m->ops[index];
+  if (op.kind != OP_ATTNBLK) return fail("op %d is not a fused attention block", index);
+  DevGuard g(m->device);
+  if (m->h2_stale && refresh_h2(m)) return 1;
+  FwdPlan plan;
+  if (make_plan(m, false, B, &plan)) return 1;
+  OpPlan &p = plan.ops[index];
+  if (mode == 1 && !p.attn_sample) return fail("op %d: the plan does not take the whole-sample attention kernel", index);
+  p.attn_sample = mode == 1; p.carries = -1;
+  hipStream_t st = m->stream;
+  const size_t n = (size_t)B * op.S * op.E;
+  CM_HIP(hipMemcpy(op.ab_x->d, h_x, n * sizeof(float), hipMemcpyHostToDevice));
+  const int rc = run_attn_block(m, op, plan, p, st, 0, 0);
+  const hipError_t e = hipStreamSynchronize(st);
+  if (rc) return 1;
+  if (e != hipSuccess) return fail("debug attention launch failed: %s", hipGetErrorString(e));
+  CM_HIP(hipMemcpy(h_out, op.ab_out->d, n * sizeof(float), hipMemcpyDeviceToHost));
+  if (h_part) CM_HIP(hipMemcpy(h_part, op.ab_out->part, (size_t)B * p.ns_out * op.E * 2 * sizeof(float), hipMemcpyDeviceToHost));
+  if (h_cnt) CM_HIP(hipMemcpy(h_cnt, op.ab_out->cnt, (size_t)B * p.ns_out * sizeof(float), hipMemcpyDeviceToHost));
+  return 0;
+}
+
+extern "C" int cm_debug_attn_pack(const float *w, int32_t N, int32_t K, uint16_t *halves, float *scale) {
+  if (!w || !halves || !scale || N < 16 || K < 32 || N % 16 || K % 32) return fail("bad argument");
+  *scale = h2_wscale(w, (size_t)N * K);
+  const std::vector<float> f = pack_attn_h2(w, N, K, *scale);
+  std::memcpy(halves, f.data(), f.size() * sizeof(float));
+  return 0;
+}
+
+extern "C" int cm_debug_attn_sample_ok(int32_t S, int32_t E, int32_t heads, int32_t groups) { return cm::attn_sample_ok(S, E, heads, groups) ? 1 : 0; }
 
 int cm_debug_conv_io(cm_model *m, int32_t index, int32_t mode, const float *h_in0, const float *h_in1, float *h_out, int32_t B) {
   CM_NOT_DIT(m, "cm_debug_conv_io");
@@ -2830,6 +2929,12 @@
   if (!m || !m->finalized || !flops) return fail("model not finalized");
   for (int i = 0; i < 8; ++i) flops[i] = 0;
   if (b16) for (int i = 0; i < 8; ++i) b16[i] = 0;
+  std::vector<char> h2_attn(m->ops.size(), 0);
+  {
+    const FwdPlan pl = plan_forward(m->ops, FwdCtx{m->precision, false, m->h2_stale, B});
+    for (size_t i = 0; i < m->ops.size(); ++i)
+      if (m->ops[i].kind == OP_ATTNBLK && pl.ops[i].attn_sample) h2_attn[m->ops[i].ab_qkv] = h2_attn[m->ops[i].ab_outc] = 1;
+  }
   for (const Op &op : m->ops) {
     if (op.kind == OP_ATTN) { flops[op.cls] += 4.0 * op.S * (double)op.S * op.E * B; continue; }
     if (op.kind != OP_CONV) continue;
@@ -2863,6 +2968,7 @@
         if (a.par) f = f * 8.0 / 27.0;
         if (cm::conv_zsplit_variant(a, op.MB, op.NB)) f *= a.par ? 6.0 / 8.0 : 18.0 / 27.0;
     }
+    if (h2_attn[&op - m->ops.data()]) mult16 = 3.0;
     if (b16 && mult16 > 0.0) b16[op.cls] += mult16 * f * B;
     else flops[op.cls] += f * B;
   }
diff --git a/crowdmod-ddpm-4d_amd/csrc/cm_train_host.inc b/crowdmod-ddpm-4d_amd/csrc/cm_train_host.inc
--- a/crowdmod-ddpm-4d_amd/csrc/cm_train_host.inc
+++ b/crowdmod-ddpm-4d_amd/csrc/cm_train_host.inc
@@ -161,6 +161,14 @@
   };
   std::vector<float> w, gam, bet, frag;
   for (Op &op : m->ops) {
+    if (op.kind == OP_ATTNBLK && op.d_win_h2 && op.d_wout_h2) {
+      std::vector<float> wo, fi, fo;
+      if (fetch(op.win_name, &w) || fetch(op.wout_name, &wo)) return 1;
+      attn_pack_h2(w.data(), wo.data(), op.E, &fi, &fo, &op.ab_in_oscale, &op.ab_out_oscale);
+      CM_HIP(hipMemcpy(op.d_win_h2, fi.data(), fi.size() * sizeof(float), hipMemcpyHostToDevice));
+      CM_HIP(hipMemcpy(op.d_wout_h2, fo.data(), fo.size() * sizeof(float), hipMemcpyHostToDevice));
+      continue;
+    }
     if (op.kind != OP_CONV || !(op.d_wwino_h2 || op.d_wqr_h2 || op.d_wfin_h2 || op.d_wups_h2)) continue;
     const int Co = op.ca.Co, Ci = op.ca.C0 + op.ca.C1;
     if (fetch(op.wname, &w)) return 1;
diff --git a/crowdmod-ddpm-4d_amd/native.py b/crowdmod-ddpm-4d_amd/native.py
--- a/crowdmod-ddpm-4d_amd/native.py
+++ b/crowdmod-ddpm-4d_amd/native.py
@@ -169,6 +169,42 @@
         raise NativeError(msg.decode("utf-8", "replace") if msg else f"libcrowdmod_hip call failed ({rc})")
 
 
+_HOOKS = {
+    "cm_debug_attn_block": (C.c_int, [_P, C.c_int32, C.c_int32, _P, _P, _P, _P, C.c_int32]),
+    "cm_debug_attn_pack": (C.c_int, [_P, C.c_int32, C.c_int32, _P, C.POINTER(C.c_float)]),
+    "cm_debug_attn_sample_ok": (C.c_int, [C.c_int32, C.c_int32, C.c_int32, C.c_int32]),
+}
+
+
+def hook(name: str):
+    fn = getattr(lib(), name)
+    fn.restype, fn.argtypes = _HOOKS[name]
+    return fn
+
+
+def debug_attn_block(handle, index: int, mode: int, x: np.ndarray):
+    x = np.ascontiguousarray(x, dtype=np.float32)
+    B, S, E = x.shape
+    ns = (S + 31) // 32
+    out = np.empty_like(x)
+    part = np.empty((B, ns, E, 2), np.float32)
+    cnt = np.empty((B, ns), np.float32)
+    check(hook("cm_debug_attn_block")(handle, index, mode, x.ctypes.data, out.ctypes.data, part.ctypes.data,
+                                      cnt.ctypes.data, B))
+    return out, part, cnt
+
+
+def debug_attn_pack(w: np.ndarray):
+    w = np.ascontiguousarray(w, dtype=np.float32)
+    N, K = w.shape
+    halves = np.empty(N * K * 2, np.uint16)
+    scale = C.c_float(0.0)
+    check(hook("cm_debug_attn_pack")(w.ctypes.data, N, K, halves.ctypes.data, C.byref(scale)))
+    f = halves.view(np.float16).astype(np.float32).reshape(N // 16, K // 32, 2, 4, 16, 8)
+    t = f.transpose(2, 0, 4, 1, 3, 5).reshape(2, N, K)
+    return t[0], t[1], float(scale.value)
+
+
 def device_count() -> int:
     n = C.c_int(0)
     check(lib().cm_device_count(C.byref(n)))
```

Measured after the change: 948.4 denoise-steps/s, aggregate over 1 GPU under weak scaling (every GPU advances its own batch of 64 chains per step), median of 6. 1.01x the previous value.
